# AdeeshKolluru/AdsorbDiff

Measured on AMD Instinct MI355X. Metric: sampled adsorbate sites/sec (50 denoise steps, ~200-atom slabs), higher is better.
Workload: dtype f32 (f16x3-split MFMA, fp32 accumulate; ADF_GEMM=f32 selects exact f32)

## Files before the change

adsorbdiff_amd/csrc/api.hip:

```cpp
#include <stdarg.h>
#include <stdlib.h>
#include <string.h>

#include <new>

#include "common.h"

static thread_local char g_err[512] = "";

void adf_set_error(const char* fmt, ...) {
    va_list ap;
    va_start(ap, fmt);
    vsnprintf(g_err, sizeof(g_err), fmt, ap);
    va_end(ap);
}

extern "C" const char* adf_last_error(void) { return g_err; }
extern "C" const char* adf_version(void) { return "adsorbdiff_hip 0.5.0 (gfx950)"; }

void adf_prof_begin(adf_painn* h, int cat, hipStream_t s) {
    if (!h->prof_on) return;
    if (h->prof_used + 2 > h->prof_ev->size()) {
        for (int i = 0; i < 512; ++i) {
            hipEvent_t e;
            if (hipEventCreate(&e) != hipSuccess) return;
            h->prof_ev->push_back(e);
        }
    }
    h->prof_cat->push_back(cat);
    (void)hipEventRecord((*h->prof_ev)[h->prof_used], s);
    h->prof_used += 1;
}
void adf_prof_end(adf_painn* h, hipStream_t s) {
    if (!h->prof_on || (h->prof_used & 1) == 0) return;
    (void)hipEventRecord((*h->prof_ev)[h->prof_used], s);
    h->prof_used += 1;
}

extern "C" int32_t adf_profile_enable(adf_painn_t h, int32_t on) {
    if (!h) { adf_set_error("null handle"); return ADF_EINVAL; }
    h->prof_on = on != 0;
    h->prof_used = 0;
    h->prof_cat->clear();
    ADF_HIP_CHECK(hipMemset(h->kcount, 0, 8 * sizeof(unsigned long long)));
    return ADF_OK;
}

extern "C" int32_t adf_profile_read(adf_painn_t h, float* ms, int64_t* count, int64_t* message_ksteps, void* stream) {
    if (!h || !ms || !count) { adf_set_error("null argument"); return ADF_EINVAL; }
    ADF_HIP_CHECK(hipStreamSynchronize((hipStream_t)stream));
    if (message_ksteps) {
        unsigned long long k[8];
        ADF_HIP_CHECK(hipMemcpy(k, h->kcount, sizeof(k), hipMemcpyDeviceToHost));
        ADF_HIP_CHECK(hipMemset(h->kcount, 0, sizeof(k)));
        *message_ksteps = (int64_t)k[0];
    }
    for (int c = 0; c < ADF_PROF_NCAT; ++c) { ms[c] = 0.f; count[c] = 0; }
    const size_t pairs = h->prof_used / 2;
    for (size_t i = 0; i < pairs; ++i) {
        float t = 0.f;
        ADF_HIP_CHECK(hipEventElapsedTime(&t, (*h->prof_ev)[2 * i], (*h->prof_ev)[2 * i + 1]));
        const int c = (*h->prof_cat)[i];
        ms[c] += t;
        count[c] += 1;
    }
    h->prof_used = 0;
    h->prof_cat->clear();
    return ADF_OK;
}

template <typename T>
static int32_t dev_alloc(T** p, size_t count) {
    if (*p) { (void)hipFree(*p); *p = nullptr; }
    if (count == 0) return ADF_OK;
    hipError_t e = hipMalloc(reinterpret_cast<void**>(p), count * sizeof(T));
    if (e != hipSuccess) {
        *p = nullptr;
        (void)hipGetLastError();
        adf_set_error("hipMalloc of %zu bytes failed: %s", count * sizeof(T), hipGetErrorString(e));
        return ADF_EOOM;
    }
    return ADF_OK;
}

extern "C" int32_t adf_painn_create(const adf_painn_hparams* hp, adf_painn_t* out) {
    if (!hp || !out) { adf_set_error("null argument"); return ADF_EINVAL; }
    if (hp->hidden_channels % ADF_SLICE_CH != 0 || hp->hidden_channels < 128 || hp->hidden_channels > 1024) {
        adf_set_error("hidden_channels=%d must be a multiple of %d in [128,1024]", hp->hidden_channels, ADF_SLICE_CH);
        return ADF_EINVAL;
    }
    if (hp->num_rbf % 2 != 0 || hp->num_rbf > 128 || hp->num_rbf < 2) {
        adf_set_error("num_rbf=%d must be even and <= 128", hp->num_rbf);
        return ADF_EINVAL;
    }
    if (hp->max_neighbors < 1 || hp->max_neighbors > ADF_MAX_K) {
        adf_set_error("max_neighbors=%d must be in [1,%d]", hp->max_neighbors, ADF_MAX_K);
        return ADF_EINVAL;
    }
    if (hp->num_layers < 1 || hp->num_layers > 16 || hp->num_heads < 0 || hp->num_heads > 2) {
        adf_set_error("num_layers must be in [1,16], num_heads in [0,2]");
        return ADF_EINVAL;
    }
    adf_painn* h = new (std::nothrow) adf_painn();
    if (!h) { adf_set_error("host allocation failed"); return ADF_EOOM; }
    memset(h, 0, sizeof(*h));
    h->hp = *hp;
    h->prof_ev = new std::vector<hipEvent_t>();
    h->prof_cat = new std::vector<int>();
    hipDeviceProp_t prop;
    if (hipGetDevice(&h->device) != hipSuccess || hipGetDeviceProperties(&prop, h->device) != hipSuccess) {
        adf_set_error("no usable HIP device: %s", hipGetErrorString(hipGetLastError()));
        adf_painn_destroy(h);
        return ADF_EHIP;
    }
    h->num_cus = prop.multiProcessorCount;
    h->dist_floor = 1.0e-3f;
    {
        const char* e = getenv("ADF_INCREMENTAL");
        h->inc_on = !(e && e[0] == '0');
        const char* e2 = getenv("ADF_INC_SYNC");
        h->inc_sync = e2 && e2[0] == '1';
    }
    const int H = hp->hidden_channels, R = hp->num_rbf, L = hp->num_layers;
    int32_t st = dev_alloc(&h->rbf_pack, (size_t)L * (H / ADF_SLICE_CH) * R * 192);
    if (st == ADF_OK) st = dev_alloc(&h->rbf_bias_pack, (size_t)L * (H / ADF_SLICE_CH) * 192);
    {
        uint16_t* p16 = nullptr;
        if (st == ADF_OK) st = dev_alloc(&p16, (size_t)L * (H / ADF_SLICE_CH) * R * 192 * 2);
        h->rbf_pack16 = p16;
    }
    if (st == ADF_OK) st = dev_alloc(&h->rbf_bias_pack16, (size_t)L * (H / ADF_SLICE_CH) * 192);
    if (st == ADF_OK) st = dev_alloc(&h->rbf_scales, 16);
    if (st == ADF_OK) st = dev_alloc(&h->flags, ADF_NFLAGS);
    if (st == ADF_OK && hipMemset(h->flags, 0, sizeof(int32_t) * ADF_NFLAGS) != hipSuccess) st = ADF_EHIP;
    {
        const size_t HH = (size_t)H * H;
        const size_t per_layer = HH + 3 * HH + 2 * HH + 2 * HH + 3 * HH;
        const size_t per_head = HH + HH / 2 + 2 * HH + HH + HH / 4 + HH / 2;
        const size_t elems = (size_t)L * per_layer + (size_t)hp->num_heads * per_head;
        h->w16_bytes = elems * 2 * sizeof(uint16_t) + 4096;
        if (st == ADF_OK) st = dev_alloc(&h->w16_arena, h->w16_bytes);
        if (st == ADF_OK) st = dev_alloc(&h->w16_scales, 256);
        if (st == ADF_OK) st = dev_alloc(&h->w16_bias_perm, (size_t)L * 2 * 3 * H);
        if (st == ADF_OK) st = dev_alloc(&h->w16_scratch, 1);
        if (st == ADF_OK) st = dev_alloc(&h->wfrag_arena, h->w16_bytes);
        {
            const char* ef = getenv("ADF_FUSED_MLP");
            h->fused_mlp = ef ? atoi(ef) : 0;
            if (h->fused_mlp < 0 || h->fused_mlp > 2) h->fused_mlp = 0;
        }
        const char* e = getenv("ADF_GEMM");
        h->gemm_f32 = e && strcmp(e, "f32") == 0;
        const char* el = getenv("ADF_LIFT");
        h->lift_on = !(el && strcmp(el, "0") == 0);
        const char* e2 = getenv("ADF_MSG");
        h->msg_f32 = e2 ? strcmp(e2, "f32") == 0 : h->gemm_f32;
    }
    if (st == ADF_OK) st = dev_alloc(&h->kcount, 8);
    if (st == ADF_OK && hipMemset(h->kcount, 0, 8 * sizeof(unsigned long long)) != hipSuccess) st = ADF_EHIP;
    if (st != ADF_OK) { adf_painn_destroy(h); return st; }
    *out = h;
    return ADF_OK;
}

static void inc_free(adf_painn* h) {
    for (int l = 0; l <= ADF_MAX_LAYERS; ++l) {
        if (h->incX[l]) (void)hipFree(h->incX[l]);
        if (h->incV[l]) (void)hipFree(h->incV[l]);
        if (l < ADF_MAX_LAYERS && h->incR[l]) (void)hipFree(h->incR[l]);
        h->incX[l] = h->incV[l] = nullptr;
        if (l < ADF_MAX_LAYERS) h->incR[l] = nullptr;
    }
    void* ptrs[] = {h->inc_c0, h->inc_chg, h->inc_pend, h->inc_need, h->inc_tf, h->inc_list, h->inc_cnt, h->inc_tmp};
    for (void* p : ptrs)
        if (p) (void)hipFree(p);
    h->inc_c0 = h->inc_chg = h->inc_pend = h->inc_need = h->inc_tf = nullptr;
    h->inc_list = h->inc_cnt = nullptr; h->inc_tmp = nullptr; h->inc_tmp_bytes = 0;
    h->inc_capN = 0; h->inc_valid = false;
}

static void free_workspaces(adf_painn* h) {
    void* ptrs[] = {h->nbr_cnt, h->nbr_src, h->nbr_shift, h->deg, h->nptr, h->cursor, h->img_cnt, h->sys_slow, h->scan_tmp,
                    h->e_src, h->e_geom, h->x, h->vecA, h->vecB, h->y, h->xh, h->vv, h->cat, h->dot, h->sys, h->rec, h->lift.buf, h->mag_a, h->mag_b, h->mag_v3,
                    h->cache_d2, h->cache_cid, h->cache_cnt, h->prev_nptr, h->prev_src, h->prev_geom};
    for (void* p : ptrs)
        if (p) (void)hipFree(p);
    h->prev_nptr = h->prev_src = nullptr; h->prev_geom = nullptr; h->inc_valid = false;
    h->nbr_cnt = h->nbr_src = h->nbr_shift = h->deg = h->nptr = h->cursor = h->img_cnt = h->sys_slow = h->e_src = nullptr;
    h->scan_tmp = nullptr; h->scan_tmp_bytes = 0;
    h->e_geom = nullptr;
    h->x = h->vecA = h->vecB = h->y = h->xh = h->vv = h->cat = h->dot = h->sys = h->rec = nullptr;
    h->lift.buf = h->mag_a = h->mag_b = h->mag_v3 = nullptr; h->lift.cap = 0; h->mag_v3_valid = false;
    h->cache_d2 = nullptr; h->cache_cid = nullptr; h->cache_cnt = nullptr; h->cache_valid = false;
    h->capN = h->capB = h->capE = 0;
}

extern "C" int32_t adf_painn_destroy(adf_painn_t h) {
    if (!h) return ADF_OK;
    free_workspaces(h);
    if (h->rbf_pack) (void)hipFree(h->rbf_pack);
    if (h->rbf_bias_pack) (void)hipFree(h->rbf_bias_pack);
    if (h->rec0) (void)hipFree(h->rec0);
    inc_free(h);
    if (h->inc_cnt_host) (void)hipHostFree(h->inc_cnt_host);
    for (int i = 0; i < 2; ++i)
        if (h->inc_ev[i]) (void)hipEventDestroy((hipEvent_t)h->inc_ev[i]);
    if (h->sub_x) (void)hipFree(h->sub_x);
    if (h->sub_vec) (void)hipFree(h->sub_vec);
    if (h->sub_f) (void)hipFree(h->sub_f);
    if (h->rbf_pack16) (void)hipFree(h->rbf_pack16);
    if (h->rbf_bias_pack16) (void)hipFree(h->rbf_bias_pack16);
    if (h->rbf_scales) (void)hipFree(h->rbf_scales);
    if (h->flags) (void)hipFree(h->flags);
    if (h->kcount) (void)hipFree(h->kcount);
    if (h->w16_arena) (void)hipFree(h->w16_arena);
    if (h->wfrag_arena) (void)hipFree(h->wfrag_arena);
    if (h->w16_scales) (void)hipFree(h->w16_scales);
    if (h->w16_bias_perm) (void)hipFree(h->w16_bias_perm);
    if (h->w16_scratch) (void)hipFree(h->w16_scratch);
    if (h->oe0_buf) (void)hipFree(h->oe0_buf);
    if (h->prof_ev) { for (hipEvent_t e : *h->prof_ev) (void)hipEventDestroy(e); delete h->prof_ev; }
    delete h->prof_cat;
    delete h;
    return ADF_OK;
}

extern "C" int32_t adf_painn_set_weights(adf_painn_t h, int32_t n_weights, const void* const* w,
                                         const float* scale_factors, void* stream) {
    if (!h || !w || !scale_factors) { adf_set_error("null argument"); return ADF_EINVAL; }
    const int L = h->hp.num_layers;
    const int expect = 2 + ADF_WEIGHTS_PER_LAYER * L + ADF_WEIGHTS_PER_HEAD * h->hp.num_heads;
    if (n_weights != expect) {
        adf_set_error("expected %d weight tensors, got %d", expect, n_weights);
        return ADF_EINVAL;
    }
    for (int i = 0; i < n_weights; ++i)
        if (!w[i]) { adf_set_error("weight %d is null", i); return ADF_EINVAL; }
    auto f = [&](int i) { return reinterpret_cast<const float*>(w[i]); };
    h->emb = f(0);
    h->rbf_offset = f(1);
    int k = 2;
    for (int l = 0; l < L; ++l) {
        adf_layer_weights& lw = h->layer[l];
        lw.ln_w = f(k++); lw.ln_b = f(k++); lw.xp0_w = f(k++); lw.xp0_b = f(k++); lw.xp2_w = f(k++); lw.xp2_b = f(k++);
        lw.rbf_w = f(k++); lw.rbf_b = f(k++); lw.vp_w = f(k++); lw.xv0_w = f(k++); lw.xv0_b = f(k++);
        lw.xv2_w = f(k++); lw.xv2_b = f(k++);
        h->scale[l] = scale_factors[l];
    }
    for (int hd = 0; hd < h->hp.num_heads; ++hd)
        for (int b = 0; b < 2; ++b) {
            adf_block_weights& bw = h->head[hd][b];
            bw.vec1_w = f(k++); bw.vec2_w = f(k++); bw.un0_w = f(k++); bw.un0_b = f(k++); bw.un2_w = f(k++);
            bw.un2_b = f(k++);
        }
    ADF_TRY(adf_pack_rbf(h, (hipStream_t)stream));
    {
        hipStream_t s = (hipStream_t)stream;
        const long long H = h->hp.hidden_channels, HH = H * H;
        unsigned char* cur = h->w16_arena;
        unsigned char* fcur = h->wfrag_arena;
        int nscale = 0;
        float* bperm = h->w16_bias_perm;
        auto split = [&](const float* w, long long rows, long long K, adf_w16* out, const float* fused_bias = nullptr,
                         bool pair_perm = false) -> int32_t {
            const long long n = rows * K;
            out->hi = cur; cur += n * 2;
            out->lo = cur; cur += n * 2;
            out->inv_scale = h->w16_scales + nscale++;
            out->bias_perm = nullptr;
            out->frag = nullptr;
            if (fused_bias) {
                out->bias_perm = bperm; bperm += 3 * H;
                ADF_TRY(adf_split_weight(w, n, out, h->w16_scratch, s, (int)H, (int)H, fused_bias));
            } else if (pair_perm) {
                ADF_TRY(adf_split_weight(w, n, out, h->w16_scratch, s, (int)H, (int)H, nullptr, 2));
            } else {
                ADF_TRY(adf_split_weight(w, n, out, h->w16_scratch, s));
            }
            if (rows % 32 == 0 && K % 16 == 0) {
                out->frag = fcur; fcur += n * 4;
                ADF_TRY(adf_pack_frag(out, (int)rows, (int)K, out->frag, s));
            }
            return ADF_OK;
        };
        for (int l = 0; l < L; ++l) {
            adf_layer_weights& lw = h->layer[l];
            ADF_TRY(split(lw.xp0_w, H, H, &lw.xp0_16));
            ADF_TRY(split(lw.xp2_w, 3 * H, H, &lw.xp2_16, lw.xp2_b));
            ADF_TRY(split(lw.vp_w, 2 * H, H, &lw.vp_16, nullptr, true));
            ADF_TRY(split(lw.xv0_w, H, 2 * H, &lw.xv0_16));
            ADF_TRY(split(lw.xv2_w, 3 * H, H, &lw.xv2_16, lw.xv2_b));
        }
        for (int hd = 0; hd < h->hp.num_heads; ++hd) {
            adf_block_weights& b0 = h->head[hd][0];
            adf_block_weights& b1 = h->head[hd][1];
            ADF_TRY(split(b0.vec1_w, H, H, &b0.vec1_16));
            ADF_TRY(split(b0.vec2_w, H / 2, H, &b0.vec2_16));
            ADF_TRY(split(b0.un0_w, H, 2 * H, &b0.un0_16));
            ADF_TRY(split(b0.un2_w, H, H, &b0.un2_16));
            ADF_TRY(split(b1.vec1_w, H / 2, H / 2, &b1.vec1_16));
            ADF_TRY(split(b1.un0_w, H / 2, H, &b1.un0_16));
        }
        if ((size_t)(cur - h->w16_arena) > h->w16_bytes || (size_t)(fcur - h->wfrag_arena) > h->w16_bytes || nscale > 256) {
            adf_set_error("internal: fp16 weight arena overflow");
            return ADF_EINVAL;
        }
    }
    h->weights_set = true;
    h->rec0_valid = false;
    h->inc_valid = false;
    return ADF_OK;
}

static int32_t ensure_capacity(adf_painn* h, int64_t N, int64_t B) {
    if (N <= h->capN && B <= h->capB) return ADF_OK;
    const int64_t capN = N > h->capN ? N : h->capN;
    const int64_t capB = B > h->capB ? B : h->capB;
    ADF_HIP_CHECK(hipDeviceSynchronize());
    free_workspaces(h);
    const int64_t H = h->hp.hidden_channels, K = h->hp.max_neighbors;
    const int64_t capE = 2 * capN * K;
    int32_t st = ADF_OK;
#define ALLOC(field, count) if (st == ADF_OK) st = dev_alloc(&h->field, (size_t)(count))
    ALLOC(nbr_cnt, capN);
    ALLOC(nbr_src, capN * K);
    ALLOC(nbr_shift, capN * K);
    ALLOC(cache_d2, capN * K);
    ALLOC(cache_cid, capN * K);
    ALLOC(cache_cnt, capN);
    ALLOC(deg, capN + 1);
    ALLOC(nptr, capN + 1);
    ALLOC(cursor, capN);
    ALLOC(img_cnt, capB);
    ALLOC(sys_slow, capB);
    ALLOC(e_src, capE);
    ALLOC(e_geom, capE);
    if (h->inc_on) {
        ALLOC(prev_nptr, capN + 1);
        ALLOC(prev_src, capE);
        ALLOC(prev_geom, capE);
    }
    if (st == ADF_OK) {
        h->scan_tmp_bytes = adf_scan_temp_bytes(capN + 1);
        unsigned char* tmp = nullptr;
        st = dev_alloc(&tmp, h->scan_tmp_bytes + 16);
        h->scan_tmp = tmp;
    }
    ALLOC(x, capN * H);
    ALLOC(vecA, capN * 3 * H);
    ALLOC(vecB, capN * 3 * H);
    ALLOC(rec, (capN + 1) * 5 * H);
    ALLOC(y, capN * H);
    ALLOC(xh, capN * 3 * H);
    ALLOC(vv, capN * 6 * H);
    ALLOC(cat, capN * 2 * H);
    ALLOC(dot, capN * H);
    ALLOC(sys, capB * 16);
    ALLOC(lift.buf, capN * 3);
    ALLOC(mag_a, capN);
    ALLOC(mag_b, capN);
    ALLOC(mag_v3, capN * 3);
#undef ALLOC
    h->lift.cap = st == ADF_OK ? capN * 3 : 0;
    if (st != ADF_OK) { free_workspaces(h); return st; }
    h->capN = capN; h->capB = capB; h->capE = capE;
    return ADF_OK;
}

static int32_t check_batch(const adf_painn* h, const adf_batch* b) {
    if (!h || !b) { adf_set_error("null argument"); return ADF_EINVAL; }
    if (b->num_atoms <= 0 || b->num_systems <= 0) { adf_set_error("empty batch"); return ADF_EINVAL; }
    if (!b->pos || !b->cell || !b->batch || !b->atom_offset) { adf_set_error("null batch array"); return ADF_EINVAL; }
    for (int k = 0; k < 3; ++k)
        if (b->reps[k] < 0 || b->reps[k] > 16) { adf_set_error("reps[%d]=%d out of range", k, b->reps[k]); return ADF_EINVAL; }
    return ADF_OK;
}

static int32_t read_flags(adf_painn* h, hipStream_t s) {
    int32_t f[ADF_NFLAGS];
    ADF_HIP_CHECK(hipMemcpyAsync(f, h->flags, sizeof(f), hipMemcpyDeviceToHost, s));
    ADF_HIP_CHECK(hipMemsetAsync(h->flags, 0, sizeof(f), s));
    ADF_HIP_CHECK(hipStreamSynchronize(s));
    if (f[4]) { adf_set_error("atomic number outside [1, %d] (rows of the embedding table)", h->hp.num_elements); return ADF_EINVAL; }
    if (f[0]) { adf_set_error("a centre atom has more than %d in-cutoff candidates", ADF_MAX_CAND); return ADF_EOVERFLOW; }
    if (f[2]) { adf_set_error("edge buffer overflow"); return ADF_EOVERFLOW; }
    if (f[3]) { adf_set_error("an atom has more than %d incoming edges", ADF_MAX_INDEG); return ADF_EOVERFLOW; }
    if (f[1]) { adf_set_error("An image has no neighbors"); return ADF_ENONEIGHBOR; }
    if (f[5]) {
        adf_set_error("non-finite model output%s", h->gemm_f32 ? " (exact-f32 arithmetic: the inputs or weights are not finite)"
                      : " in f16x3 arithmetic: an activation left the fp16 range or the inputs are not finite; "
                        "adf_painn_set_arithmetic(h, 1) selects exact f32");
        return ADF_ENUMERIC;
    }
    return ADF_OK;
}

extern "C" int32_t adf_graph_set_moving(adf_painn_t h, const int32_t* moving, const int32_t* mov_idx,
                                        const int32_t* mov_off) {
    if (!h) { adf_set_error("null handle"); return ADF_EINVAL; }
    if (moving && (!mov_idx || !mov_off)) { adf_set_error("moving mask needs mov_idx and mov_off"); return ADF_EINVAL; }
    h->moving = moving; h->mov_idx = mov_idx; h->mov_off = mov_off;
    ADF_HIP_CHECK(hipMemset(h->flags, 0, sizeof(int32_t) * ADF_NFLAGS));
    h->cache_valid = false;
    h->rec0_valid = false;
    h->inc_valid = false;
    return ADF_OK;
}

extern "C" int32_t adf_graph_build(adf_painn_t h, const adf_batch* b, void* stream, int64_t* num_edges) {
    ADF_TRY(check_batch(h, b));
    ADF_TRY(ensure_capacity(h, b->num_atoms, b->num_systems));
    hipStream_t s = (hipStream_t)stream;
    ADF_TRY(adf_graph_build_impl(h, b, s));
    if (num_edges) {
        int32_t e = 0;
        ADF_HIP_CHECK(hipMemcpyAsync(&e, h->nptr + b->num_atoms, sizeof(int32_t), hipMemcpyDeviceToHost, s));
        ADF_TRY(read_flags(h, s));
        *num_edges = e;
    }
    return ADF_OK;
}

__global__ void adf_export_edges_kernel(const int32_t* nptr, const int32_t* e_src, const float4* eg, int N,
                                        int32_t* src, int32_t* dst, float* dist, float* vec, long long cap) {
    const int n = blockIdx.x * 4 + (threadIdx.x >> 6);
    if (n >= N) return;
    for (int e = nptr[n] + (threadIdx.x & 63); e < nptr[n + 1]; e += 64) {
        if (e >= cap) continue;
        if (src) src[e] = e_src[e];
        if (dst) dst[e] = n;
        const float4 q = eg[e];
        if (dist) dist[e] = q.w;
        if (vec) { vec[3 * (size_t)e] = q.x; vec[3 * (size_t)e + 1] = q.y; vec[3 * (size_t)e + 2] = q.z; }
    }
}

__global__ void adf_export_shift_kernel(const int32_t* nbr_shift, int32_t* out, long long n, int r0, int r1, int r2) {
    const long long i = (long long)blockIdx.x * blockDim.x + threadIdx.x;
    if (i >= n) return;
    const int c = nbr_shift[i];
    const int n2 = 2 * r2 + 1, n1 = 2 * r1 + 1;
    const int ia = c / (n1 * n2), rem = c - ia * (n1 * n2);
    out[3 * i] = ia - r0;
    out[3 * i + 1] = rem / n2 - r1;
    out[3 * i + 2] = rem % n2 - r2;
}

extern "C" int32_t adf_graph_export(adf_painn_t h, int32_t* nbr_count, int32_t* nbr_src, int32_t* nbr_shift,
                                    int64_t edge_capacity, int32_t* edge_src, int32_t* edge_dst, float* edge_dist,
                                    float* edge_vec, int64_t* num_edges, void* stream) {
    if (!h || h->lastN <= 0) { adf_set_error("no graph built"); return ADF_EINVAL; }
    hipStream_t s = (hipStream_t)stream;
    const int64_t N = h->lastN, K = h->hp.max_neighbors;
    if (nbr_count) ADF_HIP_CHECK(hipMemcpyAsync(nbr_count, h->nbr_cnt, sizeof(int32_t) * N, hipMemcpyDeviceToDevice, s));
    if (nbr_src) ADF_HIP_CHECK(hipMemcpyAsync(nbr_src, h->nbr_src, sizeof(int32_t) * N * K, hipMemcpyDeviceToDevice, s));
    if (nbr_shift)
        hipLaunchKernelGGL(adf_export_shift_kernel, dim3((unsigned)((N * K + 255) / 256)), dim3(256), 0, s, h->nbr_shift,
                           nbr_shift, (long long)(N * K), h->last_reps[0], h->last_reps[1], h->last_reps[2]);
    if (edge_src || edge_dst || edge_dist || edge_vec)
        hipLaunchKernelGGL(adf_export_edges_kernel, dim3((unsigned)((N + 3) / 4)), dim3(256), 0, s, h->nptr, h->e_src,
                           h->e_geom, (int)N, edge_src, edge_dst, edge_dist, edge_vec, (long long)edge_capacity);
    ADF_HIP_CHECK(hipGetLastError());
    int32_t e = 0;
    ADF_HIP_CHECK(hipMemcpyAsync(&e, h->nptr + N, sizeof(int32_t), hipMemcpyDeviceToHost, s));
    ADF_HIP_CHECK(hipStreamSynchronize(s));
    if (num_edges) *num_edges = e;
    return ADF_OK;
}

static int32_t zero_pad_rows(adf_painn* h, int N, hipStream_t s) {
    const size_t row = (size_t)5 * h->hp.hidden_channels;
    ADF_HIP_CHECK(hipMemsetAsync(h->rec + (size_t)N * row, 0, sizeof(float) * row, s));
    return ADF_OK;
}

static bool use_fused_mlp(const adf_painn* h, int rows) {
    if (h->hp.hidden_channels != 512 || h->gemm_f32 || h->fused_mlp == 0) return false;
    if (h->fused_mlp == 1) return true;
    return rows >= 2 * 64 * h->num_cus;
}

static int32_t make_records(adf_painn* h, int l, int n, const float* x, const float* vec, bool vec_is_zero, float* rec,
                            const int32_t* row_map, hipStream_t s) {
    const int H = h->hp.hidden_channels;
    const adf_layer_weights& w = h->layer[l];
    if (n <= 0) return ADF_OK;
    adf_prof_begin(h, ADF_PROF_NODE, s);
    const bool lift = h->lift_on && !h->gemm_f32;
    static int emit = -1;
    if (emit < 0) { const char* e = getenv("ADF_LIFT_EMIT"); emit = (e && atoi(e) == 0) ? 0 : 1; }
    const bool em = lift && emit;
    ADF_TRY(adf_nodewise_layernorm(x, w.ln_w, w.ln_b, h->y, n, H, s, em ? h->mag_a : nullptr, h->rows_dev));
    if (use_fused_mlp(h, n) && (em || !lift)) {
        adf_epi ep = {};
        ep.vec_in = vec; ep.rec = rec ? rec : h->rec; ep.H = H; ep.vec_is_zero = vec_is_zero ? 1 : 0;
        ep.row_map = row_map; ep.m_dev = h->rows_dev; ep.lift_y = lift ? 1 : 0;
        ep.rec_rows = row_map ? (long long)h->inc_capN : (long long)n;
        ADF_TRY(adf_launch_mlp16(h->y, nullptr, H, em ? h->mag_a : nullptr, w.xp0_16.frag, &w.xp0_16, w.xp0_b, w.xp2_16.frag, &w.xp2_16, n,
                                 H, 1, &ep, s));
        adf_prof_end(h, s);
        return ADF_OK;
    }
    ADF_TRY(adf_linear(h, h->y, H, w.xp0_w, &w.xp0_16, w.xp0_b, h->cat, H, n, H, H, 1, s, em ? h->mag_a : nullptr,
                       em ? h->mag_b : nullptr));
    if (h->gemm_f32) {
        if (row_map) { adf_set_error("internal: mapped records need the f16x3 path"); return ADF_EINVAL; }
        ADF_TRY(adf_launch_gemm(h->cat, H, w.xp2_w, H, w.xp2_b, h->xh, 3 * H, n, 3 * H, H, 0, s));
        ADF_TRY(adf_pack_records(h, n, h->xh, vec, vec_is_zero, s, rec));
    } else {
        adf_epi ep = {};
        ep.vec_in = vec; ep.rec = rec ? rec : h->rec; ep.H = H; ep.vec_is_zero = vec_is_zero ? 1 : 0;
        ep.row_map = row_map;
        ep.rmag = em ? h->mag_b : nullptr;
        ep.m_dev = h->rows_dev;
        ADF_TRY(adf_launch_gemm16_fused(h->cat, H, &w.xp2_16, n, H, H, 1, &ep, s, lift ? &h->lift : nullptr));
    }
    adf_prof_end(h, s);
    return ADF_OK;
}

static int32_t message_layer(adf_painn* h, int l, int N, const float* x, const float* vec, float* x_out,
                             float* vec_out, bool vec_is_zero, hipStream_t s, const int32_t* tlist = nullptr,
                             int n_targets = 0, float* rec = nullptr, bool records_ready = false) {
    if (!records_ready) ADF_TRY(make_records(h, l, N, x, vec, vec_is_zero, rec, nullptr, s));
    adf_prof_begin(h, ADF_PROF_MESSAGE, s);
    const int32_t st = adf_message_impl(h, l, N, x, h->xh, vec, x_out, vec_out, vec_is_zero, s, tlist, n_targets, rec,
                                        tlist ? h->rows_dev : nullptr);
    adf_prof_end(h, s);
    return st;
}

static int32_t update_layer(adf_painn* h, int l, int N, float* x, float* vec, hipStream_t s) {
    const int H = h->hp.hidden_channels;
    const adf_layer_weights& w = h->layer[l];
    adf_prof_begin(h, ADF_PROF_NODE, s);
    if (h->gemm_f32) {
        ADF_TRY(adf_launch_gemm(vec, H, w.vp_w, H, nullptr, h->vv, 2 * H, 3 * N, 2 * H, H, 0, s));
        ADF_TRY(adf_nodewise_update_prep(h->vv, x, h->cat, h->dot, N, H, s));
        ADF_TRY(adf_linear(h, h->cat, 2 * H, w.xv0_w, &w.xv0_16, w.xv0_b, h->y, H, N, H, 2 * H, 1, s));
    } else {
        adf_epi ep = {};
        ep.v1 = h->vv; ep.dotw = h->dot; ep.cat = h->cat; ep.H = H; ep.m_dev = h->rows_dev;
        const adf_lift* lf = h->lift_on ? &h->lift : nullptr;
        ADF_TRY(adf_launch_gemm16_fused(vec, H, &w.vp_16, N, H, H, 3, &ep, s, lf));
        if (use_fused_mlp(h, N)) {
            const float* rm = nullptr;
            if (lf) {
                if (N > lf->cap) { adf_set_error("mlp16: lift scratch holds %lld rows, need %d", lf->cap, N); return ADF_EINVAL; }
                ADF_TRY(adf_launch_rowmag(x, H, H, h->cat, H, N, lf->buf, s, h->rows_dev, 1));
                rm = lf->buf;
            }
            adf_epi e2 = {};
            e2.x = x; e2.vec = vec; e2.dot = h->dot; e2.vv = h->vv; e2.scale = h->scale[l]; e2.H = H;
            e2.m_dev = h->rows_dev; e2.lift_y = h->lift_on ? 1 : 0;
            const int32_t stf = adf_launch_mlp16(x, h->cat, H, rm, w.xv0_16.frag, &w.xv0_16, w.xv0_b, w.xv2_16.frag, &w.xv2_16, N, H, 2, &e2, s);
            adf_prof_end(h, s);
            return stf;
        }
        ADF_TRY(adf_launch_gemm16(x, H, &w.xv0_16, w.xv0_b, h->y, H, N, H, 2 * H, 1, s, h->cat, H, lf, nullptr,
                                  h->lift_on ? h->mag_b : nullptr, h->rows_dev));
    }
    int32_t st;
    if (h->gemm_f32) {
        ADF_TRY(adf_launch_gemm(h->y, H, w.xv2_w, H, w.xv2_b, h->xh, 3 * H, N, 3 * H, H, 0, s));
        st = adf_nodewise_update_apply(h->xh, h->dot, h->vv, x, vec, h->scale[l], N, H, s);
    } else {
        adf_epi ep = {};
        ep.x = x; ep.vec = vec; ep.dot = h->dot; ep.vv = h->vv; ep.scale = h->scale[l]; ep.H = H;
        ep.rmag = h->lift_on ? h->mag_b : nullptr;
        ep.m_dev = h->rows_dev;
        st = adf_launch_gemm16_fused(h->y, H, &w.xv2_16, N, H, H, 2, &ep, s);
    }
    adf_prof_end(h, s);
    return st;
}

extern "C" int32_t adf_painn_message_layer(adf_painn_t h, int32_t layer, int32_t N, const float* x, const float* vec,
                                           float* x_out, float* vec_out, void* stream) {
    if (!h || !h->weights_set || layer < 0 || layer >= h->hp.num_layers || N != h->lastN) {
        adf_set_error("message_layer: bad handle/layer, or N differs from the built graph");
        return ADF_EINVAL;
    }
    hipStream_t s = (hipStream_t)stream;
    ADF_TRY(zero_pad_rows(h, N, s));
    ADF_TRY(message_layer(h, layer, N, x, vec, x_out, vec_out, false, s));
    return ADF_OK;
}

extern "C" int32_t adf_painn_update_layer(adf_painn_t h, int32_t layer, int32_t N, float* x, float* vec, void* stream) {
    if (!h || !h->weights_set || layer < 0 || layer >= h->hp.num_layers) {
        adf_set_error("update_layer: bad handle/layer");
        return ADF_EINVAL;
    }
    ADF_TRY(ensure_capacity(h, N, 1));
    return update_layer(h, layer, N, x, vec, (hipStream_t)stream);
}

__global__ void adf_scatter_rows3_kernel(const float* __restrict__ src, const int32_t* __restrict__ idx, int n,
                                         float* __restrict__ dst) {
    const int i = blockIdx.x * blockDim.x + threadIdx.x;
    if (i < 3 * n) dst[(size_t)idx[i / 3] * 3 + i % 3] = src[i];
}

static int32_t forward_impl(adf_painn_t h, const adf_batch* b, const int32_t* out_idx, int32_t n_out, float* f1,
                            float* f2, void* stream, bool head1_only = false);

extern "C" int32_t adf_painn_forward(adf_painn_t h, const adf_batch* b, float* f1, float* f2, void* stream) {
    return forward_impl(h, b, nullptr, 0, f1, f2, stream);
}

extern "C" int32_t adf_painn_forward_subset(adf_painn_t h, const adf_batch* b, const int32_t* out_idx, int32_t n_out,
                                            float* f1, float* f2, void* stream) {
    if (!out_idx || n_out < 0) { adf_set_error("forward_subset: null index list"); return ADF_EINVAL; }
    return forward_impl(h, b, out_idx, n_out, f1, f2, stream);
}

static int inc_prepare(adf_painn* h, int N) {
    const int L = h->hp.num_layers, H = h->hp.hidden_channels;
    if (!h->inc_on || !h->moving || h->gemm_f32 || h->msg_f32 || L > ADF_MAX_LAYERS || !h->prev_nptr)
        return 0;
    if (N > h->inc_capN) {
        (void)hipDeviceSynchronize();
        inc_free(h);
        const size_t cap = (size_t)N;
        int32_t st = ADF_OK;
        for (int l = 0; l <= L && st == ADF_OK; ++l) {
            st = dev_alloc(&h->incX[l], cap * H);
            if (st == ADF_OK && l >= 1) st = dev_alloc(&h->incV[l], cap * 3 * H);
            if (st == ADF_OK && l < L) st = dev_alloc(&h->incR[l], (cap + 1) * 5 * H);
        }
        if (st == ADF_OK) st = dev_alloc(&h->inc_c0, cap);
        if (st == ADF_OK) st = dev_alloc(&h->inc_chg, 2 * cap);
        if (st == ADF_OK) st = dev_alloc(&h->inc_pend, cap * L);
        if (st == ADF_OK) st = dev_alloc(&h->inc_need, cap * L);
        if (st == ADF_OK) st = dev_alloc(&h->inc_tf, cap * L);
        if (st == ADF_OK) st = dev_alloc(&h->inc_list, cap * L);
        if (st == ADF_OK) st = dev_alloc(&h->inc_cnt, (size_t)2 * ADF_MAX_LAYERS + 1);
        if (st == ADF_OK) {
            h->inc_tmp_bytes = adf_inc_temp_bytes((int64_t)cap);
            unsigned char* tmp = nullptr;
            st = dev_alloc(&tmp, h->inc_tmp_bytes + 16);
            h->inc_tmp = tmp;
        }
        if (st == ADF_OK && !h->inc_cnt_host &&
            hipHostMalloc(reinterpret_cast<void**>(&h->inc_cnt_host), sizeof(int32_t) * 2 * (2 * ADF_MAX_LAYERS + 1)) != hipSuccess)
            st = ADF_EOOM;
        for (int i = 0; i < 2 && st == ADF_OK; ++i)
            if (!h->inc_ev[i] && hipEventCreateWithFlags(reinterpret_cast<hipEvent_t*>(&h->inc_ev[i]), hipEventDisableTiming) != hipSuccess)
                st = ADF_EHIP;
        if (st != ADF_OK) {
            (void)hipGetLastError();
            inc_free(h);
            h->inc_on = false;
            fprintf(stderr, "adsorbdiff_hip: no memory for incremental layers (%d atoms), continuing without\n", N);
            return 0;
        }
        h->inc_capN = (int64_t)cap;
    }
    if (h->inc_N != N || h->inc_layers != L || h->build_serial != h->inc_serial) h->inc_valid = false;
    h->inc_N = N; h->inc_layers = L;
    int32_t* tn = h->nptr; h->nptr = h->prev_nptr; h->prev_nptr = tn;
    int32_t* ts = h->e_src; h->e_src = h->prev_src; h->prev_src = ts;
    float4* tg = h->e_geom; h->e_geom = h->prev_geom; h->prev_geom = tg;
    const int state = h->inc_valid ? 1 : 2;
    h->inc_valid = false;
    return state;
}

__global__ void adf_scatter_rows3_kernel(const float* __restrict__ src, const int32_t* __restrict__ idx, int n,
                                         float* __restrict__ dst);

static int32_t inc_harvest(adf_painn* h, int slot, bool wait, bool peek = false) {
    if (!h->inc_ev_live[slot]) return ADF_OK;
    hipEvent_t ev = (hipEvent_t)h->inc_ev[slot];
    if (wait) {
        ADF_HIP_CHECK(hipEventSynchronize(ev));
    } else {
        const hipError_t q = hipEventQuery(ev);
        if (q == hipErrorNotReady) { (void)hipGetLastError(); return ADF_OK; }
        ADF_HIP_CHECK(q);
    }
    const int L = h->inc_layers, N = h->inc_pend_N[slot];
    const int32_t* c = h->inc_cnt_host + (size_t)slot * (2 * ADF_MAX_LAYERS + 1);
    for (int i = 0; i < 2 * L + 1; ++i) h->inc_seen[i] = c[i];
    h->inc_seen_valid = true;
    h->inc_pend_Nseen = N;
    if (peek) return ADF_OK;
    h->inc_ev_live[slot] = false;
    for (int l = 0; l < L; ++l) {
        const bool whole = h->inc_pend_whole[slot][l] != 0;
        h->inc_rows += (unsigned long long)(whole ? N : c[l]);
        h->inc_rows_full += (unsigned long long)N;
        h->inc_edges += (unsigned long long)(whole ? c[2 * L] : c[L + l]);
        if (whole || c[l] > 0) ++h->inc_launches;
    }
    return ADF_OK;
}

static int32_t forward_incremental(adf_painn* h, int N, const int32_t* Z, const int32_t* out_idx, int32_t n_out,
                                   float* f1, float* f2, bool first, int heads, hipStream_t s) {
    const int L = h->hp.num_layers, H = h->hp.hidden_channels;
    const size_t cap = (size_t)h->inc_capN, row = (size_t)5 * H;
    if (out_idx && n_out == 0) return ADF_OK;
    adf_prof_begin(h, ADF_PROF_GRAPH, s);
    if (first) {
        ADF_TRY(adf_nodewise_embed(h, Z, N, h->incX[0], s));
        for (int l = 0; l < L; ++l) ADF_HIP_CHECK(hipMemsetAsync(h->incR[l] + (size_t)N * row, 0, sizeof(float) * row, s));
        ADF_HIP_CHECK(hipMemsetAsync(h->inc_pend, 0, cap * L, s));
    } else {
        ADF_TRY(adf_inc_compare(h, N, s));
    }
    ADF_HIP_CHECK(hipMemsetAsync(h->inc_cnt, 0, sizeof(int32_t) * (2 * ADF_MAX_LAYERS + 1), s));
    if (out_idx) ADF_TRY(adf_inc_need_from_list(h, N, L, out_idx, n_out, s));
    for (int l = 0; l < L; ++l) ADF_TRY(adf_inc_plan_layer(h, l, N, first, out_idx != nullptr, s));
    ADF_HIP_CHECK(hipMemcpyAsync(h->inc_cnt + 2 * L, h->nptr + N, sizeof(int32_t), hipMemcpyDeviceToDevice, s));
    const int slot = h->inc_slot;
    h->inc_slot ^= 1;
    if (h->inc_ev_live[slot]) ADF_TRY(inc_harvest(h, slot, true));
    int32_t* host = h->inc_cnt_host + (size_t)slot * (2 * ADF_MAX_LAYERS + 1);
    ADF_HIP_CHECK(hipMemcpyAsync(host, h->inc_cnt, sizeof(int32_t) * (2 * L + 1), hipMemcpyDeviceToHost, s));
    ADF_HIP_CHECK(hipEventRecord((hipEvent_t)h->inc_ev[slot], s));
    h->inc_ev_live[slot] = true;
    h->inc_pend_N[slot] = N;
    ADF_TRY(inc_harvest(h, slot ^ 1, false));
    if (h->inc_sync) ADF_TRY(inc_harvest(h, slot, true, true));
    adf_prof_end(h, s);
    if (first) ADF_TRY(make_records(h, 0, N, h->incX[0], nullptr, true, h->incR[0], nullptr, s));
    for (int l = 0; l < L; ++l) {
        const int n_seen = h->inc_seen_valid ? h->inc_seen[l] : N;
        const bool whole = first || !h->inc_seen_valid || h->inc_pend_Nseen != N || (long long)n_seen * 10 >= (long long)N * 9;
        h->inc_pend_whole[slot][l] = whole ? 1 : 0;
        if (h->inc_sync && !whole && n_seen == 0) continue;
        const float* vin = l == 0 ? h->vecA : h->incV[l];
        if (whole) {
            ADF_TRY(message_layer(h, l, N, h->incX[l], vin, h->incX[l + 1], h->incV[l + 1], l == 0, s, nullptr, 0,
                                  h->incR[l], true));
            ADF_TRY(update_layer(h, l, N, h->incX[l + 1], h->incV[l + 1], s));
            if (l + 1 < L)
                ADF_TRY(make_records(h, l + 1, N, h->incX[l + 1], h->incV[l + 1], false, h->incR[l + 1], nullptr, s));
            continue;
        }
        const int32_t* list = h->inc_list + cap * l;
        const int ncap = h->inc_sync ? n_seen : N;
        h->rows_dev = h->inc_cnt + l;
        int32_t st = message_layer(h, l, N, h->incX[l], vin, h->x, h->vecB, l == 0, s, list, ncap, h->incR[l], true);
        if (st == ADF_OK) st = update_layer(h, l, ncap, h->x, h->vecB, s);
        if (st == ADF_OK) {
            adf_prof_begin(h, ADF_PROF_NODE, s);
            st = adf_inc_scatter_rows(h->x, list, ncap, H, h->incX[l + 1], s, h->rows_dev);
            if (st == ADF_OK) st = adf_inc_scatter_rows(h->vecB, list, ncap, 3 * H, h->incV[l + 1], s, h->rows_dev);
            adf_prof_end(h, s);
        }
        if (st == ADF_OK && l + 1 < L) st = make_records(h, l + 1, ncap, h->x, h->vecB, false, h->incR[l + 1], list, s);
        h->rows_dev = nullptr;
        ADF_TRY(st);
    }
    adf_prof_begin(h, ADF_PROF_HEADS, s);
    if (!out_idx) {
        if (heads >= 1) ADF_TRY(adf_head_forward(h, 0, N, h->incX[L], h->incV[L], f1, s));
        if (heads == 2) ADF_TRY(adf_head_forward(h, 1, N, h->incX[L], h->incV[L], f2, s));
        h->x_last = h->incX[L];
    } else {
        if (n_out > h->capS) {
            const int64_t c = (int64_t)n_out + n_out / 4 + 64;
            if (h->sub_x) (void)hipFree(h->sub_x);
            if (h->sub_vec) (void)hipFree(h->sub_vec);
            if (h->sub_f) (void)hipFree(h->sub_f);
            h->sub_x = h->sub_vec = h->sub_f = nullptr; h->capS = 0;
            ADF_TRY(dev_alloc(&h->sub_x, (size_t)c * H));
            ADF_TRY(dev_alloc(&h->sub_vec, (size_t)c * 3 * H));
            ADF_TRY(dev_alloc(&h->sub_f, (size_t)c * 3));
            h->capS = c;
        }
        ADF_TRY(adf_inc_gather_rows(h->incX[L], out_idx, n_out, H, h->sub_x, s));
        ADF_TRY(adf_inc_gather_rows(h->incV[L], out_idx, n_out, 3 * H, h->sub_vec, s));
        for (int hd = 0; hd < heads; ++hd) {
            ADF_TRY(adf_head_forward(h, hd, n_out, h->sub_x, h->sub_vec, h->sub_f, s));
            hipLaunchKernelGGL(adf_scatter_rows3_kernel, dim3((3 * n_out + 255) / 256), dim3(256), 0, s, h->sub_f, out_idx,
                               n_out, hd == 0 ? f1 : f2);
        }
        ADF_HIP_CHECK(hipGetLastError());
    }
    adf_prof_end(h, s);
    h->inc_valid = true;
    return ADF_OK;
}

static int32_t forward_impl(adf_painn_t h, const adf_batch* b, const int32_t* out_idx, int32_t n_out, float* f1,
                            float* f2, void* stream, bool head1_only) {
    ADF_TRY(check_batch(h, b));
    if (!h->weights_set) { adf_set_error("weights not set"); return ADF_EINVAL; }
    const int heads = head1_only ? 1 : h->hp.num_heads;
    if (heads > h->hp.num_heads) { adf_set_error("the model has no force head"); return ADF_EINVAL; }
    if (!b->atomic_numbers || (heads >= 1 && !f1) || (heads == 2 && !f2)) { adf_set_error("null argument"); return ADF_EINVAL; }
    h->x_last = nullptr;
    hipStream_t s = (hipStream_t)stream;
    const int N = b->num_atoms;
    ADF_TRY(ensure_capacity(h, N, b->num_systems));
    const int inc = inc_prepare(h, N);
    adf_prof_begin(h, ADF_PROF_GRAPH, s);
    ADF_TRY(adf_graph_build_impl(h, b, s));
    adf_prof_end(h, s);
    if (inc) {
        h->inc_serial = h->build_serial;
        return forward_incremental(h, N, b->atomic_numbers, out_idx, n_out, f1, f2, inc == 2, heads, s);
    }
    ADF_TRY(zero_pad_rows(h, N, s));
    ADF_TRY(adf_nodewise_embed(h, b->atomic_numbers, N, h->x, s));
    float* vin = h->vecA;
    float* vout = h->vecB;
    const int L = h->hp.num_layers, H = h->hp.hidden_channels;
    float* rec0 = nullptr;
    bool rec0_ready = false;
    if (h->moving) {
        const size_t row = (size_t)5 * H;
        if ((int64_t)N + 1 > h->rec0_cap) {
            if (h->rec0) { (void)hipFree(h->rec0); h->rec0 = nullptr; }
            h->rec0_cap = 0; h->rec0_valid = false;
            ADF_TRY(dev_alloc(&h->rec0, ((size_t)N + 1) * row));
            h->rec0_cap = (int64_t)N + 1;
        }
        rec0 = h->rec0;
        rec0_ready = h->rec0_valid && h->rec0_N == N;
        if (!rec0_ready) ADF_HIP_CHECK(hipMemsetAsync(rec0 + (size_t)N * row, 0, sizeof(float) * row, s));
        h->rec0_valid = true; h->rec0_N = N;
    }
    if (!out_idx) {
        for (int l = 0; l < L; ++l) {
            if (l == 0) ADF_TRY(message_layer(h, 0, N, h->x, vin, h->x, vout, true, s, nullptr, 0, rec0, rec0_ready));
            else
            ADF_TRY(message_layer(h, l, N, h->x, vin, h->x, vout, l == 0, s));
            ADF_TRY(update_layer(h, l, N, h->x, vout, s));
            float* t = vin; vin = vout; vout = t;
        }
        adf_prof_begin(h, ADF_PROF_HEADS, s);
        if (heads >= 1) ADF_TRY(adf_head_forward(h, 0, N, h->x, vin, f1, s));
        if (heads == 2) ADF_TRY(adf_head_forward(h, 1, N, h->x, vin, f2, s));
        adf_prof_end(h, s);
        h->x_last = h->x;
        return ADF_OK;
    }
    if (n_out == 0) return ADF_OK;
    if (n_out > h->capS) {
        const int64_t cap = (int64_t)n_out + n_out / 4 + 64;
        if (h->sub_x) (void)hipFree(h->sub_x);
        if (h->sub_vec) (void)hipFree(h->sub_vec);
        if (h->sub_f) (void)hipFree(h->sub_f);
        h->sub_x = h->sub_vec = h->sub_f = nullptr; h->capS = 0;
        ADF_TRY(dev_alloc(&h->sub_x, (size_t)cap * H));
        ADF_TRY(dev_alloc(&h->sub_vec, (size_t)cap * 3 * H));
        ADF_TRY(dev_alloc(&h->sub_f, (size_t)cap * 3));
        h->capS = cap;
    }
    for (int l = 0; l + 1 < L; ++l) {
        if (l == 0) ADF_TRY(message_layer(h, 0, N, h->x, vin, h->x, vout, true, s, nullptr, 0, rec0, rec0_ready));
        else
        ADF_TRY(message_layer(h, l, N, h->x, vin, h->x, vout, l == 0, s));
        ADF_TRY(update_layer(h, l, N, h->x, vout, s));
        float* t = vin; vin = vout; vout = t;
    }
    ADF_TRY(message_layer(h, L - 1, N, h->x, vin, h->sub_x, h->sub_vec, L == 1, s, out_idx, n_out,
                          L == 1 ? rec0 : nullptr, L == 1 && rec0_ready));
    ADF_TRY(update_layer(h, L - 1, n_out, h->sub_x, h->sub_vec, s));
    adf_prof_begin(h, ADF_PROF_HEADS, s);
    for (int hd = 0; hd < heads; ++hd) {
        ADF_TRY(adf_head_forward(h, hd, n_out, h->sub_x, h->sub_vec, h->sub_f, s));
        hipLaunchKernelGGL(adf_scatter_rows3_kernel, dim3((3 * n_out + 255) / 256), dim3(256), 0, s, h->sub_f, out_idx,
                           n_out, hd == 0 ? f1 : f2);
    }
    ADF_HIP_CHECK(hipGetLastError());
    adf_prof_end(h, s);
    return ADF_OK;
}

extern "C" int32_t adf_painn_set_energy_head(adf_painn_t h, int32_t n_weights, const void* const* w, void* stream) {
    if (!h || !w) { adf_set_error("null argument"); return ADF_EINVAL; }
    if (n_weights != 4) { adf_set_error("set_energy_head: expected 4 tensors (out_energy.0.weight/bias, out_energy.2.weight/bias), got %d", n_weights); return ADF_EINVAL; }
    for (int i = 0; i < 4; ++i)
        if (!w[i]) { adf_set_error("energy-head tensor %d is null", i); return ADF_EINVAL; }
    const int H = h->hp.hidden_channels, H2 = H / 2;
    const size_t n = (size_t)H2 * H;
    if (!h->oe0_buf) ADF_TRY(dev_alloc(&h->oe0_buf, n * 4 + 64));
    h->oe0_w = reinterpret_cast<const float*>(w[0]);
    h->oe0_b = reinterpret_cast<const float*>(w[1]);
    h->oe2_w = reinterpret_cast<const float*>(w[2]);
    h->oe2_b = reinterpret_cast<const float*>(w[3]);
    adf_w16& e = h->oe0_16;
    e = adf_w16{};
    e.hi = h->oe0_buf; e.lo = h->oe0_buf + n * 2; e.inv_scale = reinterpret_cast<float*>(h->oe0_buf + n * 4);
    ADF_TRY(adf_split_weight(h->oe0_w, (long long)n, &e, reinterpret_cast<unsigned int*>(h->oe0_buf + n * 4 + 16),
                             (hipStream_t)stream));
    h->energy_set = true;
    return ADF_OK;
}

extern "C" int32_t adf_painn_set_distance_floor(adf_painn_t h, float floor) {
    if (!h || !(floor > 0.f)) { adf_set_error("set_distance_floor: null handle or non-positive floor"); return ADF_EINVAL; }
    if (floor != h->dist_floor) {
        h->dist_floor = floor;
        h->cache_valid = false;
        h->rec0_valid = false;
        h->inc_valid = false;
    }
    return ADF_OK;
}

__global__ __launch_bounds__(256) void adf_energy_sum_kernel(const float* __restrict__ y, int H2, const float* __restrict__ w,
                                                             const float* __restrict__ bias, const int32_t* __restrict__ atom_offset,
                                                             float* __restrict__ energy) {
    __shared__ float part[4];
    const int b = blockIdx.x, lane = threadIdx.x & 63, wave = threadIdx.x >> 6;
    const int a0 = atom_offset[b], a1 = atom_offset[b + 1];
    const float b0 = bias[0];
    float acc = 0.f;
    for (int a = a0 + wave; a < a1; a += 4) {
        const float* row = y + (size_t)a * H2;
        float d = 0.f;
        for (int c = lane; c < H2; c += 64) d = fmaf(row[c], w[c], d);
        for (int o = 32; o > 0; o >>= 1) d = __fadd_rn(d, __shfl_xor(d, o, 64));
        acc = __fadd_rn(acc, __fadd_rn(d, b0));
    }
    if (lane == 0) part[wave] = acc;
    __syncthreads();
    if (threadIdx.x == 0) energy[b] = __fadd_rn(__fadd_rn(part[0], part[1]), __fadd_rn(part[2], part[3]));
}

extern "C" int32_t adf_painn_forward_energy(adf_painn_t h, const adf_batch* b, float* energy, float* forces, void* stream) {
    ADF_TRY(check_batch(h, b));
    if (!h->energy_set) { adf_set_error("forward_energy: energy head not set (adf_painn_set_energy_head)"); return ADF_EINVAL; }
    if (!energy || (h->hp.num_heads >= 1 && !forces)) { adf_set_error("forward_energy: null output"); return ADF_EINVAL; }
    if (h->hp.num_heads > 1) { adf_set_error("forward_energy: the S2EF model has one force head"); return ADF_EINVAL; }
    hipStream_t s = (hipStream_t)stream;
    ADF_TRY(forward_impl(h, b, nullptr, 0, forces, nullptr, stream));
    if (!h->x_last) { adf_set_error("internal: no node features after the forward"); return ADF_EINVAL; }
    const int N = b->num_atoms, H = h->hp.hidden_channels, H2 = H / 2;
    adf_prof_begin(h, ADF_PROF_HEADS, s);
    ADF_TRY(adf_linear(h, h->x_last, H, h->oe0_w, &h->oe0_16, h->oe0_b, h->y, H2, N, H2, H, 1, s));
    hipLaunchKernelGGL(adf_energy_sum_kernel, dim3(b->num_systems), dim3(256), 0, s, h->y, H2, h->oe2_w, h->oe2_b,
                       b->atom_offset, energy);
    ADF_HIP_CHECK(hipGetLastError());
    adf_prof_end(h, s);
    return ADF_OK;
}

extern "C" int32_t adf_linear_forward(const float* A, const float* W, const float* bias, float* C, int32_t M,
                                      int32_t N, int32_t K, int32_t act_ssilu, int32_t mode, void* stream) {
    hipStream_t s = (hipStream_t)stream;
    if (!A || !W || !C || M <= 0 || N <= 0 || K <= 0) { adf_set_error("bad argument"); return ADF_EINVAL; }
    if (mode == 0) return adf_launch_gemm(A, K, W, K, bias, C, N, M, N, K, act_ssilu, s);
    unsigned char* buf = nullptr;
    const size_t n = (size_t)N * K;
    ADF_TRY(dev_alloc(&buf, n * 4 + 64));
    adf_w16 w16 = {};
    w16.hi = buf; w16.lo = buf + n * 2; w16.inv_scale = reinterpret_cast<float*>(buf + n * 4);
    unsigned int* scratch = reinterpret_cast<unsigned int*>(buf + n * 4 + 16);
    int32_t st = adf_split_weight(W, (long long)n, &w16, scratch, s);
    float* mags = nullptr;
    const char* el = getenv("ADF_LIFT");
    const bool lift = !(el && strcmp(el, "0") == 0);
    if (st == ADF_OK && lift) st = dev_alloc(&mags, (size_t)M);
    adf_lift lf = {mags, M};
    if (st == ADF_OK) st = adf_launch_gemm16(A, K, &w16, bias, C, N, M, N, K, act_ssilu, s, nullptr, 0, lift ? &lf : nullptr);
    (void)hipStreamSynchronize(s);
    (void)hipFree(buf);
    if (mags) (void)hipFree(mags);
    return st;
}

extern "C" int32_t adf_painn_set_arithmetic(adf_painn_t h, int32_t exact_f32) {
    if (!h) { adf_set_error("null handle"); return ADF_EINVAL; }
    h->gemm_f32 = exact_f32 != 0;
    h->msg_f32 = exact_f32 != 0;
    h->rec0_valid = false;
    h->inc_valid = false;
    return ADF_OK;
}

extern "C" int32_t adf_painn_set_fused_mlp(adf_painn_t h, int32_t mode) {
    if (!h || mode < 0 || mode > 2) { adf_set_error("set_fused_mlp: mode must be 0 (never), 1 (always) or 2 (by size)"); return ADF_EINVAL; }
    h->fused_mlp = mode;
    return ADF_OK;
}

extern "C" int32_t adf_painn_set_incremental(adf_painn_t h, int32_t on) {
    if (!h) { adf_set_error("null handle"); return ADF_EINVAL; }
    if ((on != 0) != h->inc_on) {
        ADF_HIP_CHECK(hipDeviceSynchronize());
        h->inc_on = on != 0;
        if (!h->inc_on) inc_free(h);
        if (h->inc_on && h->capN > 0 && !h->prev_nptr) {
            int32_t st = dev_alloc(&h->prev_nptr, (size_t)h->capN + 1);
            if (st == ADF_OK) st = dev_alloc(&h->prev_src, (size_t)h->capE);
            if (st == ADF_OK) st = dev_alloc(&h->prev_geom, (size_t)h->capE);
            if (st != ADF_OK) { h->inc_on = false; return st; }
        }
    }
    h->inc_valid = false;
    (void)inc_harvest(h, h->inc_slot, true);
    (void)inc_harvest(h, h->inc_slot ^ 1, true);
    h->inc_seen_valid = false;
    h->inc_rows = h->inc_rows_full = h->inc_edges = h->inc_launches = 0;
    return ADF_OK;
}

extern "C" int32_t adf_check_flags(adf_painn_t h, void* stream) {
    if (!h) { adf_set_error("null handle"); return ADF_EINVAL; }
    return read_flags(h, (hipStream_t)stream);
}

static int32_t model_check(void* h, const adf_batch* b) { return check_batch((adf_painn*)h, b); }
static int32_t model_grow(void* h, const adf_batch* b, float** sys) {
    adf_painn* p = (adf_painn*)h;
    ADF_TRY(ensure_capacity(p, b->num_atoms, b->num_systems));
    *sys = p->sys;
    return ADF_OK;
}
static int32_t model_forward(void* h, const adf_batch* b, const int32_t* out_idx, int32_t n_out, float* f1, float* f2,
                             hipStream_t s) {
    return forward_impl((adf_painn*)h, b, out_idx, out_idx ? n_out : 0, f1, f2, s, !f2);
}
static void model_prof(void* h, bool begin, hipStream_t s) {
    if (begin) adf_prof_begin((adf_painn*)h, ADF_PROF_STEPPER, s);
    else adf_prof_end((adf_painn*)h, s);
}
static adf_model model(adf_painn_t h) { return {h, model_check, model_grow, model_forward, model_prof}; }

extern "C" int32_t adf_sde_init_placement(adf_painn_t h, const adf_batch* b, float* pos, const int32_t* tags,
                                          const float* noise, void* stream) {
    return adf_model_init_placement(model(h), b, pos, tags, noise, (hipStream_t)stream);
}

extern "C" int32_t adf_sde_step(adf_painn_t h, const adf_batch* b, float* pos, const int32_t* tags,
                                const int32_t* fixed, const float* f1, const float* f2, const adf_step_coef* coef,
                                const float* z_tr, const float* z_rot, int32_t early_stop_count, int32_t* state,
                                float* dcom, float* drot, void* stream) {
    return adf_model_sde_step(model(h), b, pos, tags, fixed, f1, f2, coef, nullptr, 0, z_tr, z_rot, early_stop_count, state,
                              dcom, drot, (hipStream_t)stream);
}

extern "C" int32_t adf_sde_step_scheduled(adf_painn_t h, const adf_batch* b, float* pos, const int32_t* tags,
                                          const int32_t* fixed, const float* f1, const float* f2,
                                          const adf_step_coef* coefs_dev, int32_t num_steps, const float* z_tr,
                                          const float* z_rot, int32_t early_stop_count, int32_t* state, float* dcom,
                                          float* drot, void* stream) {
    return adf_model_sde_step(model(h), b, pos, tags, fixed, f1, f2, nullptr, coefs_dev, num_steps, z_tr, z_rot,
                              early_stop_count, state, dcom, drot, (hipStream_t)stream);
}

extern "C" int32_t adf_sample(adf_painn_t h, const adf_batch* b, float* pos, const int32_t* tags, const int32_t* fixed,
                              const adf_step_coef* coefs_dev, int32_t num_steps, const float* z_tr_all,
                              const float* z_rot_all, int32_t early_stop_count, int32_t poll_every, int32_t* state,
                              const int32_t* out_idx, int32_t n_out, float* f1, float* f2, void* stream) {
    return adf_model_sample(model(h), b, pos, tags, fixed, coefs_dev, num_steps, z_tr_all, z_rot_all, early_stop_count,
                            poll_every, state, out_idx, n_out, f1, f2, nullptr, 0, (hipStream_t)stream);
}

extern "C" int32_t adf_sample_traj(adf_painn_t h, const adf_batch* b, float* pos, const int32_t* tags, const int32_t* fixed,
                                   const adf_step_coef* coefs_dev, int32_t num_steps, const float* z_tr_all,
                                   const float* z_rot_all, int32_t early_stop_count, int32_t poll_every, int32_t* state,
                                   const int32_t* out_idx, int32_t n_out, float* f1, float* f2, adf_frames_t sink,
                                   int32_t frame_every, void* stream) {
    if (!sink) { adf_set_error("sample_traj: null sink"); return ADF_EINVAL; }
    return adf_model_sample(model(h), b, pos, tags, fixed, coefs_dev, num_steps, z_tr_all, z_rot_all, early_stop_count,
                            poll_every, state, out_idx, n_out, f1, f2, sink, frame_every, (hipStream_t)stream);
}

extern "C" int32_t adf_tr_step(adf_painn_t h, const adf_batch* b, float* pos, const int32_t* tags, const float* f1,
                               const adf_tr_coef* coef, const adf_tr_coef* coefs_dev, int32_t num_steps, const float* z,
                               int32_t early_stop_count, int32_t* state, float* dcom, void* stream) {
    return adf_model_tr_step(model(h), b, pos, tags, f1, coef, coefs_dev, num_steps, z, early_stop_count, state, dcom,
                             (hipStream_t)stream);
}

extern "C" int32_t adf_tr_sample(adf_painn_t h, const adf_batch* b, float* pos, const int32_t* tags,
                                 const adf_tr_coef* coefs_dev, int32_t num_steps, const float* z_all,
                                 int32_t early_stop_count, int32_t poll_every, int32_t* state, const int32_t* out_idx,
                                 int32_t n_out, float* f1, void* stream) {
    return adf_model_tr_sample(model(h), b, pos, tags, coefs_dev, num_steps, z_all, early_stop_count, poll_every, state,
                               out_idx, n_out, f1, nullptr, 0, (hipStream_t)stream);
}

extern "C" int32_t adf_tr_sample_traj(adf_painn_t h, const adf_batch* b, float* pos, const int32_t* tags,
                                      const adf_tr_coef* coefs_dev, int32_t num_steps, const float* z_all,
                                      int32_t early_stop_count, int32_t poll_every, int32_t* state, const int32_t* out_idx,
                                      int32_t n_out, float* f1, adf_frames_t sink, int32_t frame_every, void* stream) {
    if (!sink) { adf_set_error("tr_sample_traj: null sink"); return ADF_EINVAL; }
    return adf_model_tr_sample(model(h), b, pos, tags, coefs_dev, num_steps, z_all, early_stop_count, poll_every, state,
                               out_idx, n_out, f1, sink, frame_every, (hipStream_t)stream);
}

extern "C" int32_t adf_get_counters(adf_painn_t h, adf_counters* out, void* stream) {
    if (!h || !out || h->lastN <= 0) { adf_set_error("no forward has run"); return ADF_EINVAL; }
    hipStream_t s = (hipStream_t)stream;
    const int64_t N = h->lastN, H = h->hp.hidden_channels, R = h->hp.num_rbf, L = h->hp.num_layers;
    int32_t e = 0;
    ADF_HIP_CHECK(hipMemcpyAsync(&e, h->nptr + N, sizeof(int32_t), hipMemcpyDeviceToHost, s));
    ADF_HIP_CHECK(hipStreamSynchronize(s));
    const int64_t E = e;
    out->num_edges = E;
    out->num_atoms = N;
    out->message_bytes_per_layer = E * (3 * H * 4 + 12 + 8) + N * (3 * H * 4 + 3 * H * 4) + N * (H * 4 + 3 * H * 4);
    const int64_t head = 2 * (3 * N * H * H + 3 * N * H * H / 2 + N * 2 * H * H + N * H * H + 3 * N * (H / 2) * (H / 2) +
                              N * H * H / 2);
    out->dense_flops = L * (30 * H * H * N + 2 * R * 3 * H * E) + h->hp.num_heads * head;
    ADF_TRY(inc_harvest(h, h->inc_slot, true));
    ADF_TRY(inc_harvest(h, h->inc_slot ^ 1, true));
    out->inc_rows = (int64_t)h->inc_rows; out->inc_rows_full = (int64_t)h->inc_rows_full;
    out->inc_msg_launches = (int64_t)h->inc_launches; out->inc_msg_edges = (int64_t)h->inc_edges;
    return ADF_OK;
}
```

adsorbdiff_amd/csrc/common.h:

```cpp
#pragma once
#include <hip/hip_runtime.h>
#include <stdint.h>
#include <stdio.h>
#include <string>
#include <vector>

#include "../../include/adsorbdiff_hip.h"

#define ADF_GROUP_NODES 32
#define ADF_SLICE_CH 64
#define ADF_MAX_CAND 1024
#define ADF_MAX_K 128
#define ADF_NFLAGS 8
#define ADF_MAX_INDEG 1024
#define ADF_MAX_LAYERS 16

void adf_set_error(const char* fmt, ...);

#define ADF_HIP_CHECK(expr)                                                             \
    do {                                                                                \
        hipError_t _e = (expr);                                                         \
        if (_e != hipSuccess) {                                                         \
            adf_set_error("%s failed: %s (%s:%d)", #expr, hipGetErrorString(_e),        \
                          __FILE__, __LINE__);                                          \
            return (_e == hipErrorOutOfMemory) ? ADF_EOOM : ADF_EHIP;                   \
        }                                                                               \
    } while (0)

#define ADF_TRY(expr)                     \
    do {                                  \
        int32_t _s = (expr);              \
        if (_s != ADF_OK) return _s;      \
    } while (0)

struct adf_w16 {
    void* hi;
    void* lo;
    float* inv_scale;
    float* bias_perm;
    void* frag;
};
struct adf_epi {
    const float* vec_in;
    float* rec;
    float* x;
    float* vec;
    const float* dot;
    const float* vv;
    float* v1;
    float* dotw;
    float* cat;
    float scale;
    int H;
    int vec_is_zero;
    const float* A2;
    int K1;
    const int32_t* row_map;
    const float* rmag;
    unsigned int* out_mag;
    const int32_t* m_dev;
    int accumulate;
    int lift_y;
    const float* gate;
    int gate_ld;
    long long rec_rows;
};
struct adf_lift {
    float* buf;
    long long cap;
};
struct adf_layer_weights {
    const float *ln_w, *ln_b, *xp0_w, *xp0_b, *xp2_w, *xp2_b, *rbf_w, *rbf_b;
    const float *vp_w, *xv0_w, *xv0_b, *xv2_w, *xv2_b;
    adf_w16 xp0_16, xp2_16, vp_16, xv0_16, xv2_16;
};
struct adf_block_weights {
    const float *vec1_w, *vec2_w, *un0_w, *un0_b, *un2_w, *un2_b;
    adf_w16 vec1_16, vec2_16, un0_16, un2_16;
};

struct adf_painn {
    adf_painn_hparams hp;
    int device;
    bool weights_set;
    const float* emb;
    const float* rbf_offset;
    adf_layer_weights layer[16];
    adf_block_weights head[2][2];
    float scale[16];
    float* rbf_pack;
    float* rbf_bias_pack;
    void* rbf_pack16;
    float* rbf_bias_pack16;
    float* rbf_scales;
    unsigned char* w16_arena;
    size_t w16_bytes;
    float* w16_scales;
    float* w16_bias_perm;
    unsigned int* w16_scratch;
    unsigned char* wfrag_arena;
    int fused_mlp;
    bool gemm_f32;
    bool msg_f32;
    bool lift_on;
    adf_lift lift;
    float *mag_a, *mag_b;
    float* mag_v3;
    bool mag_v3_valid;

    int64_t capN, capB, capE;
    int32_t* nbr_cnt;
    int32_t* nbr_src;
    int32_t* nbr_shift;
    int32_t* deg;
    int32_t* nptr;
    int32_t* cursor;
    int32_t* img_cnt;
    int32_t* sys_slow;
    void* scan_tmp;
    size_t scan_tmp_bytes;
    const int32_t* moving;
    const int32_t* mov_idx;
    const int32_t* mov_off;
    float* cache_d2;
    int32_t* cache_cid;
    int32_t* cache_cnt;
    bool cache_valid;
    int32_t* e_src;
    float4* e_geom;
    int32_t* flags;
    float *x, *vecA, *vecB, *y, *xh, *vv, *cat, *dot;
    float* rec;
    bool rbf_uniform;
    float* rec0;
    int64_t rec0_cap, rec0_N;
    bool rec0_valid;
    bool inc_on;
    bool inc_valid;
    int64_t inc_capN, inc_N;
    int inc_layers;
    float* incX[ADF_MAX_LAYERS + 1];
    float* incV[ADF_MAX_LAYERS + 1];
    float* incR[ADF_MAX_LAYERS];
    int32_t *prev_nptr, *prev_src;
    float4* prev_geom;
    unsigned char *inc_c0, *inc_chg;
    unsigned char *inc_pend, *inc_need, *inc_tf;
    int32_t* inc_list;
    int32_t* inc_cnt;
    int32_t* inc_cnt_host;
    void* inc_ev[2];
    bool inc_ev_live[2];
    int inc_slot;
    bool inc_sync;
    int32_t inc_seen[2 * ADF_MAX_LAYERS + 1];
    bool inc_seen_valid;
    unsigned char inc_pend_whole[2][ADF_MAX_LAYERS];
    int32_t inc_pend_N[2];
    int32_t inc_pend_Nseen;
    const int32_t* rows_dev;
    void* inc_tmp; size_t inc_tmp_bytes;
    unsigned long long inc_rows, inc_rows_full, inc_edges, inc_launches;
    unsigned long long build_serial, inc_serial;
    float *sub_x, *sub_vec, *sub_f;
    int64_t capS;
    float* sys;
    const float *oe0_w, *oe0_b, *oe2_w, *oe2_b;
    adf_w16 oe0_16;
    unsigned char* oe0_buf;
    bool energy_set;
    const float* x_last;
    float dist_floor;
    int64_t lastN, lastB;
    int32_t last_reps[3];
    int num_cus;
    bool prof_on;
    std::vector<hipEvent_t>* prof_ev;
    std::vector<int>* prof_cat;
    size_t prof_used;
    unsigned long long* kcount;
};

enum { ADF_PROF_GRAPH = 0, ADF_PROF_MESSAGE = 1, ADF_PROF_NODE = 2, ADF_PROF_HEADS = 3, ADF_PROF_STEPPER = 4 };
void adf_prof_begin(adf_painn* h, int cat, hipStream_t s);
void adf_prof_end(adf_painn* h, hipStream_t s);

int32_t adf_launch_gemm(const float* A, int lda, const float* W, int ldw, const float* bias, float* C, int ldc,
                        int M, int N, int K, int act_ssilu, hipStream_t s);
int32_t adf_launch_gemm16(const float* A, int lda, const adf_w16* W, const float* bias, float* C, int ldc, int M,
                          int N, int K, int act_ssilu, hipStream_t s, const float* A2 = nullptr, int K1 = 0,
                          const adf_lift* lf = nullptr, const float* premag = nullptr, float* out_mag = nullptr,
                          const int32_t* m_dev = nullptr, int accumulate = 0,
                          const float* gate = nullptr, int gate_ld = 0);
int32_t adf_launch_rowmag(const float* A, int lda, int K1, const float* A2, int K2, long long M, float* mag, hipStream_t s,
                          const int32_t* m_dev = nullptr, int m_mul = 1);
int32_t adf_split_weight(const float* w, long long n, adf_w16* out, unsigned int* scratch_bits, hipStream_t s,
                         int perm_H = 0, int K = 0, const float* bias = nullptr, int parts = 3);
int32_t adf_launch_gemm16_vecnorm(const float* A, int lda, const adf_w16* W, float* nrm, int M, int N, int K,
                                  hipStream_t s, const adf_lift* lf = nullptr, const float* premag = nullptr);
int32_t adf_launch_gemm16_fused(const float* A, int lda, const adf_w16* W, int M, int H, int K, int epi,
                                const adf_epi* ep, hipStream_t s, const adf_lift* lf = nullptr);
static inline int32_t adf_linear(const adf_painn* h, const float* A, int lda, const float* W, const adf_w16* W16,
                                 const float* bias, float* C, int ldc, int M, int N, int K, int act, hipStream_t s,
                                 const float* premag = nullptr, float* out_mag = nullptr) {
    if (h->gemm_f32) return adf_launch_gemm(A, lda, W, K, bias, C, ldc, M, N, K, act, s);
    return adf_launch_gemm16(A, lda, W16, bias, C, ldc, M, N, K, act, s, nullptr, 0, h->lift_on ? &h->lift : nullptr,
                             h->lift_on ? premag : nullptr, h->lift_on ? out_mag : nullptr, h->rows_dev);
}
int32_t adf_pack_frag(const adf_w16* w, int N, int K, void* out, hipStream_t s);
int32_t adf_launch_mlp16(const float* A1, const float* A2, int lda, const float* rmag, const void* W0f, const adf_w16* W0,
                         const float* bias0, const void* W2f, const adf_w16* W2, int M, int H, int epi, const adf_epi* ep,
                         hipStream_t s);
int32_t adf_graph_build_impl(adf_painn* h, const adf_batch* b, hipStream_t s);
size_t adf_inc_temp_bytes(int64_t n);
int32_t adf_inc_compare(adf_painn* h, int N, hipStream_t s);
int32_t adf_inc_need_from_list(adf_painn* h, int N, int L, const int32_t* out_idx, int n_out, hipStream_t s);
int32_t adf_inc_plan_layer(adf_painn* h, int l, int N, bool first, bool have_need, hipStream_t s);
int32_t adf_inc_scatter_rows(const float* src, const int32_t* idx, int n, int width, float* dst, hipStream_t s,
                             const int32_t* n_dev = nullptr);
int32_t adf_inc_gather_rows(const float* src, const int32_t* idx, int n, int width, float* dst, hipStream_t s);
size_t adf_scan_temp_bytes(int64_t n);
int32_t adf_message_impl(adf_painn* h, int layer, int N, const float* x, const float* xh, const float* vec,
                         float* x_out, float* vec_out, bool vec_is_zero, hipStream_t s,
                         const int32_t* tlist = nullptr, int n_targets = 0, const float* rec = nullptr,
                         const int32_t* n_targets_dev = nullptr);
int32_t adf_pack_rbf(adf_painn* h, hipStream_t s);
int32_t adf_pack_rbf_layer(adf_painn* h, int l, hipStream_t s);
int32_t adf_pack_records(adf_painn* h, int N, const float* xh, const float* vec, bool vec_is_zero, hipStream_t s,
                         float* rec = nullptr);
int32_t adf_nodewise_embed(adf_painn* h, const int32_t* Z, int N, float* x, hipStream_t s);
int32_t adf_nodewise_layernorm(const float* x, const float* w, const float* b, float* y, int N, int H, hipStream_t s,
                               float* out_mag = nullptr, const int32_t* n_dev = nullptr);
int32_t adf_nodewise_update_prep(const float* vv, const float* x, float* cat, float* dot, int N, int H, hipStream_t s);
int32_t adf_nodewise_update_apply(const float* h3, const float* dot, const float* vv, float* x, float* vec,
                                  float scale, int N, int H, hipStream_t s);
int32_t adf_head_forward(adf_painn* h, int head, int N, const float* x, const float* vec, float* out, hipStream_t s);
int32_t adf_stepper_init(const adf_batch* b, float* pos, const int32_t* tags, const float* noise,
                         hipStream_t s);
int32_t adf_stepper_step(float* sys, const adf_batch* b, float* pos, const int32_t* tags, const int32_t* fixed,
                         const float* f1, const float* f2, const adf_step_coef* coef, const adf_step_coef* coefs_dev,
                         int num_steps, const float* z_tr, const float* z_rot, int32_t early_stop_count,
                         int32_t* state, float* dcom, float* drot, hipStream_t s);
int32_t adf_stepper_tr_step(float* sys, const adf_batch* b, float* pos, const int32_t* tags, const float* f1,
                            const adf_tr_coef* coef, const adf_tr_coef* coefs_dev, int num_steps, const float* z,
                            int32_t early_stop_count, int32_t* state, float* dcom, hipStream_t s);

struct adf_model {
    void* h;
    int32_t (*check)(void* h, const adf_batch* b);
    int32_t (*grow)(void* h, const adf_batch* b, float** sys);
    int32_t (*forward)(void* h, const adf_batch* b, const int32_t* out_idx, int32_t n_out, float* f1, float* f2,
                       hipStream_t s);
    void (*prof)(void* h, bool begin, hipStream_t s);
};
int32_t adf_frames_push_impl(adf_frames* f, const float* src, hipStream_t s);
int32_t adf_model_init_placement(const adf_model& m, const adf_batch* b, float* pos, const int32_t* tags,
                                 const float* noise, hipStream_t s);
int32_t adf_model_sde_step(const adf_model& m, const adf_batch* b, float* pos, const int32_t* tags, const int32_t* fixed,
                           const float* f1, const float* f2, const adf_step_coef* coef, const adf_step_coef* coefs_dev,
                           int32_t num_steps, const float* z_tr, const float* z_rot, int32_t early_stop_count,
                           int32_t* state, float* dcom, float* drot, hipStream_t s);
int32_t adf_model_tr_step(const adf_model& m, const adf_batch* b, float* pos, const int32_t* tags, const float* f1,
                          const adf_tr_coef* coef, const adf_tr_coef* coefs_dev, int32_t num_steps, const float* z,
                          int32_t early_stop_count, int32_t* state, float* dcom, hipStream_t s);
int32_t adf_model_sample(const adf_model& m, const adf_batch* b, float* pos, const int32_t* tags, const int32_t* fixed,
                         const adf_step_coef* coefs_dev, int32_t num_steps, const float* z_tr_all, const float* z_rot_all,
                         int32_t early_stop_count, int32_t poll_every, int32_t* state, const int32_t* out_idx,
                         int32_t n_out, float* f1, float* f2, adf_frames* sink, int32_t frame_every, hipStream_t s);
int32_t adf_model_tr_sample(const adf_model& m, const adf_batch* b, float* pos, const int32_t* tags,
                            const adf_tr_coef* coefs_dev, int32_t num_steps, const float* z_all, int32_t early_stop_count,
                            int32_t poll_every, int32_t* state, const int32_t* out_idx, int32_t n_out, float* f1,
                            adf_frames* sink, int32_t frame_every, hipStream_t s);
```

adsorbdiff_amd/csrc/gemm16.hip:

```cpp
#include <stdlib.h>

#include "common.h"

typedef float f32x16 __attribute__((ext_vector_type(16)));
typedef _Float16 half8 __attribute__((ext_vector_type(8)));
typedef _Float16 half4 __attribute__((ext_vector_type(4)));

#ifndef EPI_ABL
#define EPI_ABL 0
#endif
#ifndef G16_ABL
#define G16_ABL 0
#endif
#ifndef G16_WDEEP
#define G16_WDEEP 1
#endif
#define HK 32
#define TLD3 96
#define TLD2 64
#define HLD 40

__device__ __forceinline__ float adf_pow2_lift(float mx) {
    if (!(mx > 0.f) || !(mx < 3.0e38f)) return 1.0f;
    int e;
    (void)frexpf(mx, &e);
    e = 15 - e;
    e = e > 120 ? 120 : (e < -120 ? -120 : e);
    return ldexpf(1.0f, e);
}

__device__ __forceinline__ float ssilu16(float x) {
    float s = x / (1.0f + expf(-x));
    return s * 1.6666666666666667f;
}

__device__ __forceinline__ float adf_row16_max(float v) {
#define ADF_ROR(n_) __int_as_float(__builtin_amdgcn_update_dpp(0, __float_as_int(v), 0x120 + (n_), 0xf, 0xf, false))
    v = fmaxf(v, ADF_ROR(8));
    v = fmaxf(v, ADF_ROR(4));
    v = fmaxf(v, ADF_ROR(2));
    v = fmaxf(v, ADF_ROR(1));
#undef ADF_ROR
    return v;
}

template <int ACT, int MI, int NJ, int EPI, bool WR = false, int NWN = 2>
__global__ __launch_bounds__(128 * NWN, (MI == 4 || NWN == 4 ? 1 : 2)) void adf_gemm_f16x3_kernel(
    const float* __restrict__ A, int lda, const _Float16* __restrict__ Whi, const _Float16* __restrict__ Wlo,
    const float* __restrict__ inv_scale, const float* __restrict__ bias, float* __restrict__ C, int ldc, int Mh, int N,
    int K, int tiles_n, adf_epi ep) {
    const int M = ep.m_dev ? min(Mh, (int)*ep.m_dev) : Mh;
    static_assert(NWN == 2 || WR, "eight waves only with the register-streamed weights");
    constexpr int NT = 128 * NWN;
    constexpr int TM = 64 * MI;
    constexpr int TN = 32 * NJ * NWN;
    constexpr int NA = TM * 8 / NT;
    static_assert(TM * 8 % NT == 0, "A staging: whole float4s per thread");
    constexpr int LDS_WR = 4 * TM * HLD > NT / 64 * 6400 ? 4 * TM * HLD : NT / 64 * 6400;
    __shared__ __attribute__((aligned(16))) _Float16 lds[WR ? LDS_WR : (2 * TM + 2 * TN) * HLD];
    __shared__ float rinv[TM];
    _Float16* Ahi = lds;
    _Float16* Alo = Ahi + TM * HLD;
    _Float16* Bhi = Alo + TM * HLD;
    _Float16* Blo = Bhi + TN * HLD;
    const int tid = threadIdx.x;
    const int lane = tid & 63;
    const int wave = tid >> 6;
    const int wm = (wave / NWN) * (32 * MI);
    const int wn = (wave % NWN) * (32 * NJ);

    const int id = blockIdx.x;
    const int xcd = id & 7;
    const int qd = id >> 3;
    const int tile_m = (qd / tiles_n) * 8 + xcd;
    const int tile_n = qd % tiles_n;
    const int m0 = tile_m * (EPI >= 3 ? TM / 3 : TM);
    const int n0 = tile_n * TN;
    if (m0 >= M) return;

    unsigned int a_goff[NA];
    int a_off[NA];
    float a_rs[NA];
    auto global_row = [&](int row) -> unsigned int {
        if constexpr (EPI >= 3) {
            const int atom = m0 + (row / 96) * 32 + (row & 31), ax = (row % 96) >> 5;
            return (unsigned int)min(atom, M - 1) * 3u + ax;
        } else {
            return (unsigned int)min(m0 + row, M - 1);
        }
    };
#pragma unroll
    for (int i = 0; i < NA; ++i) {
        const int f = tid + NT * i;
        const int row = f >> 3, kq = f & 7;
        const unsigned int grow = global_row(row);
        a_goff[i] = (grow * (unsigned int)lda + kq * 4) * 4u;
        a_off[i] = row * HLD + kq * 4;
        a_rs[i] = ep.rmag ? adf_pow2_lift(ep.rmag[grow]) : 1.0f;
    }
    if (tid < TM) rinv[tid] = ep.rmag ? 1.0f / adf_pow2_lift(ep.rmag[global_row(tid)]) : 1.0f;
    const char* const A1b = reinterpret_cast<const char*>(A);
    const char* const A2b = reinterpret_cast<const char*>(ep.A2) - (size_t)ep.K1 * 4;
    int w_src[NJ];
    int w_off[NJ];
#pragma unroll
    for (int i = 0; i < NJ; ++i) {
        const int f = tid + 256 * i;
        const int row = f >> 2, part = f & 3;
        w_src[i] = min(n0 + row, N - 1) * K + part * 8;
        w_off[i] = row * HLD + part * 8;
    }

    float4 ra[NA];
    half8 rwh[NJ], rwl[NJ];
#pragma unroll
    for (int i = 0; i < NA; ++i) ra[i] = *reinterpret_cast<const float4*>(A1b + a_goff[i]);
    if constexpr (!WR) {
#pragma unroll
        for (int i = 0; i < NJ; ++i) {
            rwh[i] = *reinterpret_cast<const half8*>(Whi + w_src[i]);
            rwl[i] = *reinterpret_cast<const half8*>(Wlo + w_src[i]);
        }
    }
    half8 wfa[NJ][2], wfb[NJ][2];
    const half8* const wfr = reinterpret_cast<const half8*>(Whi) + (size_t)((n0 + wn) / 32) * (K / 16) * 128 + lane;
    auto load_wf = [&](int s_, half8 (&wf)[NJ][2]) {
#pragma unroll
        for (int j = 0; j < NJ; ++j) {
            const size_t base = ((size_t)j * (K / 16) + s_) * 128;
            wf[j][0] = wfr[base];
            wf[j][1] = wfr[base + 64];
        }
    };
    if constexpr (WR) load_wf(0, wfa);

    f32x16 acc[MI][NJ];
#pragma unroll
    for (int i = 0; i < MI; ++i)
#pragma unroll
        for (int j = 0; j < NJ; ++j)
#pragma unroll
            for (int r = 0; r < 16; ++r) acc[i][j][r] = 0.f;

    const int nk = K / HK;
    const int fa = (wm + (lane & 31)) * HLD + (lane >> 5) * 8;
    const int fb = (wn + (lane & 31)) * HLD + (lane >> 5) * 8;
    auto stage_a = [&](int boff = 0) {
#pragma unroll
        for (int i = 0; i < NA; ++i) {
            if (G16_ABL & 2) {
                *reinterpret_cast<float2*>(Ahi + boff + a_off[i]) = make_float2(ra[i].x, ra[i].y);
                *reinterpret_cast<float2*>(Alo + boff + a_off[i]) = make_float2(ra[i].z, ra[i].w);
                continue;
            }
            const float sx = ra[i].x * a_rs[i], sy = ra[i].y * a_rs[i], sz = ra[i].z * a_rs[i], sw = ra[i].w * a_rs[i];
            half4 h, l;
            h[0] = (_Float16)sx; h[1] = (_Float16)sy; h[2] = (_Float16)sz; h[3] = (_Float16)sw;
            l[0] = (_Float16)(sx - (float)h[0]); l[1] = (_Float16)(sy - (float)h[1]);
            l[2] = (_Float16)(sz - (float)h[2]); l[3] = (_Float16)(sw - (float)h[3]);
            *reinterpret_cast<half4*>(Ahi + boff + a_off[i]) = h;
            *reinterpret_cast<half4*>(Alo + boff + a_off[i]) = l;
        }
    };
    auto request_a = [&](int kt1) {
        const int k1 = kt1 * HK;
        const char* ab = ((ep.K1 > 0 && k1 >= ep.K1) ? A2b : A1b) + (size_t)k1 * 4;
#pragma unroll
        for (int i = 0; i < NA; ++i) ra[i] = *reinterpret_cast<const float4*>(ab + ((G16_ABL & 4) ? (a_goff[i] & 127u) : a_goff[i]));
    };
    if constexpr (WR) {
        auto kstep = [&](int boff, int ks, const half8 (&cur)[NJ][2]) {
            if (G16_ABL & 8) { asm volatile("" :: "v"(cur[0][0]), "v"(cur[0][1]), "v"(cur[NJ - 1][0]), "v"(cur[NJ - 1][1])); return; }
#pragma unroll
            for (int i = 0; i < MI; ++i) {
                const half8 ah = *reinterpret_cast<const half8*>(Ahi + boff + fa + i * 32 * HLD + ks * 16);
                const half8 al = *reinterpret_cast<const half8*>(Alo + boff + fa + i * 32 * HLD + ks * 16);
#pragma unroll
                for (int j = 0; j < NJ; ++j) {
                    acc[i][j] = __builtin_amdgcn_mfma_f32_32x32x16_f16(al, cur[j][0], acc[i][j], 0, 0, 0);
                    acc[i][j] = __builtin_amdgcn_mfma_f32_32x32x16_f16(ah, cur[j][1], acc[i][j], 0, 0, 0);
                    acc[i][j] = __builtin_amdgcn_mfma_f32_32x32x16_f16(ah, cur[j][0], acc[i][j], 0, 0, 0);
                }
            }
        };
        {
            constexpr int BUF = 2 * TM * HLD;
            float4 rb[NA];
            auto request_b = [&](int kt1) {
                const int k1 = kt1 * HK;
                const char* ab = ((ep.K1 > 0 && k1 >= ep.K1) ? A2b : A1b) + (size_t)k1 * 4;
#pragma unroll
                for (int i = 0; i < NA; ++i) rb[i] = *reinterpret_cast<const float4*>(ab + ((G16_ABL & 4) ? (a_goff[i] & 127u) : a_goff[i]));
            };
            auto stage_from = [&](const float4 (&src)[NA], int boff) {
#pragma unroll
                for (int i = 0; i < NA; ++i) {
                    if (G16_ABL & 2) {
                        *reinterpret_cast<float2*>(Ahi + boff + a_off[i]) = make_float2(src[i].x, src[i].y);
                        *reinterpret_cast<float2*>(Alo + boff + a_off[i]) = make_float2(src[i].z, src[i].w);
                        continue;
                    }
                    const float sx = src[i].x * a_rs[i], sy = src[i].y * a_rs[i], sz = src[i].z * a_rs[i], sw = src[i].w * a_rs[i];
                    half4 h, l;
                    h[0] = (_Float16)sx; h[1] = (_Float16)sy; h[2] = (_Float16)sz; h[3] = (_Float16)sw;
                    l[0] = (_Float16)(sx - (float)h[0]); l[1] = (_Float16)(sy - (float)h[1]);
                    l[2] = (_Float16)(sz - (float)h[2]); l[3] = (_Float16)(sw - (float)h[3]);
                    *reinterpret_cast<half4*>(Ahi + boff + a_off[i]) = h;
                    *reinterpret_cast<half4*>(Alo + boff + a_off[i]) = l;
                }
            };
#if G16_WDEEP
            half8 wfc[NJ][2], wfd[NJ][2];
            load_wf(1, wfb);
            auto tile = [&](int kt, int cur, const float4 (&nxt_regs)[NA], const half8 (&w0)[NJ][2], const half8 (&w1)[NJ][2],
                            half8 (&w2)[NJ][2], half8 (&w3)[NJ][2]) {
                load_wf(min(2 * kt + 2, 2 * nk - 1), w2);
                __builtin_amdgcn_sched_barrier(0);
                kstep(cur, 0, w0);
                __builtin_amdgcn_sched_barrier(0);
                load_wf(min(2 * kt + 3, 2 * nk - 1), w3);
                __builtin_amdgcn_sched_barrier(0);
                kstep(cur, 1, w1);
                stage_from(nxt_regs, BUF - cur);
#else
            auto tile = [&](int kt, int cur, const float4 (&nxt_regs)[NA]) {
                load_wf(2 * kt + 1, wfb);
                __builtin_amdgcn_sched_barrier(0);
                kstep(cur, 0, wfa);
                __builtin_amdgcn_sched_barrier(0);
                load_wf(min(2 * kt + 2, 2 * nk - 1), wfa);
                __builtin_amdgcn_sched_barrier(0);
                kstep(cur, 1, wfb);
                stage_from(nxt_regs, BUF - cur);
#endif
                __builtin_amdgcn_sched_group_barrier(0x100, 2 * MI, 0);
#pragma unroll
                for (int u = 0; u < 3 * MI * NJ; ++u) {
                    __builtin_amdgcn_sched_group_barrier(0x8, 1, 0);
                    __builtin_amdgcn_sched_group_barrier(0x2, 4, 0);
                    if (u % 3 == 2) __builtin_amdgcn_sched_group_barrier(0x200, 1, 0);
                }
                __builtin_amdgcn_sched_barrier(0);
            };
            __syncthreads();
            stage_a(0);
            request_a(min(1, nk - 1));
            request_b(min(2, nk - 1));
            __syncthreads();
            for (int kt = 0; kt < nk; kt += 2) {
#if G16_WDEEP
                tile(kt, 0, ra, wfa, wfb, wfc, wfd);
                request_a(min(kt + 3, nk - 1));
                __syncthreads();
                tile(kt + 1, BUF, rb, wfc, wfd, wfa, wfb);
#else
                tile(kt, 0, ra);
                request_a(min(kt + 3, nk - 1));
                __syncthreads();
                tile(kt + 1, BUF, rb);
#endif
                request_b(min(kt + 4, nk - 1));
                __syncthreads();
            }
        }
    } else {
    for (int kt = 0; kt < nk; ++kt) {
        __syncthreads();
        stage_a();
#pragma unroll
        for (int i = 0; i < NJ; ++i) {
            *reinterpret_cast<half8*>(Bhi + w_off[i]) = rwh[i];
            *reinterpret_cast<half8*>(Blo + w_off[i]) = rwl[i];
        }
        __syncthreads();
        if (kt + 1 < nk) {
            const int k1 = (kt + 1) * HK;
            request_a(kt + 1);
#pragma unroll
            for (int i = 0; i < NJ; ++i) {
                rwh[i] = *reinterpret_cast<const half8*>(Whi + w_src[i] + k1);
                rwl[i] = *reinterpret_cast<const half8*>(Wlo + w_src[i] + k1);
            }
        }
#pragma unroll
        for (int ks = 0; ks < 2; ++ks) {
            half8 bh[NJ], bl[NJ];
#pragma unroll
            for (int j = 0; j < NJ; ++j) {
                bh[j] = *reinterpret_cast<const half8*>(Bhi + fb + j * 32 * HLD + ks * 16);
                bl[j] = *reinterpret_cast<const half8*>(Blo + fb + j * 32 * HLD + ks * 16);
            }
#pragma unroll
            for (int i = 0; i < MI; ++i) {
                const half8 ah = *reinterpret_cast<const half8*>(Ahi + fa + i * 32 * HLD + ks * 16);
                const half8 al = *reinterpret_cast<const half8*>(Alo + fa + i * 32 * HLD + ks * 16);
#pragma unroll
                for (int j = 0; j < NJ; ++j) {
                    acc[i][j] = __builtin_amdgcn_mfma_f32_32x32x16_f16(al, bh[j], acc[i][j], 0, 0, 0);
                    acc[i][j] = __builtin_amdgcn_mfma_f32_32x32x16_f16(ah, bl[j], acc[i][j], 0, 0, 0);
                    acc[i][j] = __builtin_amdgcn_mfma_f32_32x32x16_f16(ah, bh[j], acc[i][j], 0, 0, 0);
                }
            }
        }
    }
    }

    const float isc = *inv_scale;
    if constexpr (EPI == 0) {
        if (((N | ldc) & 3) == 0 && (reinterpret_cast<uintptr_t>(C) & 15) == 0 && NJ % 2 == 0) {
            const int q = lane & 31;
            __syncthreads();
            float* T = reinterpret_cast<float*>(lds) + wave * (32 * TLD2);
#pragma unroll
            for (int jj = 0; jj < NJ / 2; ++jj) {
                const int cb = n0 + wn + 64 * jj;
                const float bv0 = (bias && cb + q < N) ? bias[cb + q] : 0.f;
                const float bv1 = (bias && cb + 32 + q < N) ? bias[cb + 32 + q] : 0.f;
#pragma unroll
                for (int i = 0; i < MI; ++i) {
#pragma unroll
                    for (int r = 0; r < 16; ++r) {
                        const int lr = (r & 3) + 8 * (r >> 2) + 4 * (lane >> 5);
                        const float sc = isc * rinv[wm + 32 * i + lr];
                        float v0 = acc[i][2 * jj][r] * sc + bv0, v1 = acc[i][2 * jj + 1][r] * sc + bv1;
                        if (ACT) { v0 = ssilu16(v0); v1 = ssilu16(v1); }
                        T[lr * TLD2 + q] = v0;
                        T[lr * TLD2 + 32 + q] = v1;
                    }
                    __builtin_amdgcn_fence(__ATOMIC_RELEASE, "wavefront");
                    __builtin_amdgcn_wave_barrier();
#pragma unroll
                    for (int it = 0; it < 8; ++it) {
                        const int item = lane + 64 * it;
                        const int lr = item >> 4, c4 = item & 15;
                        const int row = m0 + wm + 32 * i + lr, col = cb + 4 * c4;
                        float4 v = *reinterpret_cast<const float4*>(T + lr * TLD2 + 4 * c4);
                        if (row < M && col < N) {
                            if (ep.gate) {
                                const float4 g4 = *reinterpret_cast<const float4*>(ep.gate + (size_t)(row / 3) * ep.gate_ld + col);
                                v.x = g4.x * v.x; v.y = g4.y * v.y; v.z = g4.z * v.z; v.w = g4.w * v.w;
                            }
                            if (ep.accumulate) {
                                const float4 o = *reinterpret_cast<const float4*>(C + (size_t)row * ldc + col);
                                v.x += o.x; v.y += o.y; v.z += o.z; v.w += o.w;
                            }
                            *reinterpret_cast<float4*>(C + (size_t)row * ldc + col) = v;
                        }
                        if (ep.out_mag) {
                            float mg = col < N ? fmaxf(fmaxf(fabsf(v.x), fabsf(v.y)), fmaxf(fabsf(v.z), fabsf(v.w))) : 0.f;
                            mg = adf_row16_max(mg);
                            if (c4 == 0 && row < M) atomicMax(ep.out_mag + row, __float_as_uint(mg));
                        }
                    }
                    __builtin_amdgcn_wave_barrier();
                }
            }
            return;
        }
#pragma unroll
        for (int j = 0; j < NJ; ++j) {
            const int col = n0 + wn + 32 * j + (lane & 31);
            if (col >= N) continue;
            const float bv = bias ? bias[col] : 0.f;
#pragma unroll
            for (int i = 0; i < MI; ++i) {
#pragma unroll
                for (int r = 0; r < 16; ++r) {
                    const int row = m0 + wm + 32 * i + (r & 3) + 8 * (r >> 2) + 4 * (lane >> 5);
                    if (row < M) {
                        float v = acc[i][j][r] * (isc * rinv[row - m0]) + bv;
                        if (ACT) v = ssilu16(v);
                        if (ep.accumulate) v += C[(size_t)row * ldc + col];
                        C[(size_t)row * ldc + col] = v;
                        if (ep.out_mag) atomicMax(ep.out_mag + row, __float_as_uint(fabsf(v)));
                    }
                }
            }
        }
    } else if constexpr (EPI == 3) {
        static_assert(EPI != 3 || (NJ == 2 && MI == 3), "vec_proj epilogue: 3 components x (v1, v2)");
        const int q = lane & 31;
        const int g = (n0 + wn) / 64;
        const int H = ep.H;
        const float inv_sqrt_h = 1.0f / sqrtf((float)H);
        __syncthreads();
        float* T = reinterpret_cast<float*>(lds) + wave * 3200;
        const int a0 = m0 + (wave / NWN) * 32;
        float dv[16], nv[16];
#pragma unroll
        for (int r = 0; r < 16; ++r) {
            const int lr = (r & 3) + 8 * (r >> 2) + 4 * (lane >> 5);
            float d = 0.f, qq = 0.f;
#pragma unroll
            for (int i = 0; i < 3; ++i) {
                const float sc = isc * rinv[wm + 32 * i + lr];
                const float v1 = acc[i][0][r] * sc, v2 = acc[i][1][r] * sc;
                d += v1 * v2;
                qq += v2 * v2;
                T[lr * TLD3 + i * 32 + q] = v1;
            }
            dv[r] = d * inv_sqrt_h;
            nv[r] = sqrtf(qq + 1e-8f);
        }
        __builtin_amdgcn_fence(__ATOMIC_RELEASE, "wavefront");
        __builtin_amdgcn_wave_barrier();
#pragma unroll
        for (int it = 0; it < 4; ++it) {
            const int item = lane + 64 * it;
            const int lr = item >> 3, c4 = item & 7;
            const int n = a0 + lr;
            if (n < M) {
                float* vo = ep.v1 + (size_t)n * 3 * H + 32 * g + 4 * c4;
#pragma unroll
                for (int ax = 0; ax < 3; ++ax) {
                    const float4 tv_ = *reinterpret_cast<const float4*>(T + lr * TLD3 + ax * 32 + 4 * c4);
                    if (G16_ABL & 1) asm volatile("" :: "v"(tv_.x), "v"(tv_.w)); else
                    *reinterpret_cast<float4*>(vo + ax * H) = tv_;
                }
            }
        }
        __builtin_amdgcn_wave_barrier();
#pragma unroll
        for (int r = 0; r < 16; ++r) {
            const int lr = (r & 3) + 8 * (r >> 2) + 4 * (lane >> 5);
            T[lr * TLD3 + q] = dv[r];
            T[lr * TLD3 + 32 + q] = nv[r];
        }
        __builtin_amdgcn_fence(__ATOMIC_RELEASE, "wavefront");
        __builtin_amdgcn_wave_barrier();
#pragma unroll
        for (int it = 0; it < 4; ++it) {
            const int lr = it * 8 + (lane >> 3), c4 = lane & 7;
            const int n = a0 + lr, c = 32 * g + 4 * c4;
            if (n < M) {
                const float4 dv_ = *reinterpret_cast<const float4*>(T + lr * TLD3 + 4 * c4);
                const float4 nv_ = *reinterpret_cast<const float4*>(T + lr * TLD3 + 32 + 4 * c4);
                if (G16_ABL & 1) { asm volatile("" :: "v"(dv_.x), "v"(nv_.w)); } else {
                *reinterpret_cast<float4*>(ep.dotw + (size_t)n * H + c) = dv_;
                *reinterpret_cast<float4*>(ep.cat + (size_t)n * H + c) = nv_;
                }
            }
        }
    } else if constexpr (EPI == 4) {
        static_assert(EPI != 4 || (NJ == 2 && MI == 3), "norm epilogue: 3 components x 64 columns per wave");
        const int q = lane & 31;
        const int cb = n0 + wn;
        __syncthreads();
        float* T = reinterpret_cast<float*>(lds) + wave * 3200;
        const int a0 = m0 + (wave / NWN) * 32;
#pragma unroll
        for (int r = 0; r < 16; ++r) {
            const int lr = (r & 3) + 8 * (r >> 2) + 4 * (lane >> 5);
#pragma unroll
            for (int j = 0; j < 2; ++j) {
                const float a = acc[0][j][r] * (isc * rinv[wm + lr]), b = acc[1][j][r] * (isc * rinv[wm + 32 + lr]),
                            d = acc[2][j][r] * (isc * rinv[wm + 64 + lr]);
                T[lr * TLD2 + j * 32 + q] = sqrtf(a * a + b * b + d * d);
            }
        }
        __builtin_amdgcn_fence(__ATOMIC_RELEASE, "wavefront");
        __builtin_amdgcn_wave_barrier();
#pragma unroll
        for (int it = 0; it < 8; ++it) {
            const int lr = it * 4 + (lane >> 4), c4 = lane & 15;
            const int n = a0 + lr, c = cb + 4 * c4;
            if (n < M && c < N)
                *reinterpret_cast<float4*>(ep.cat + (size_t)n * N + c) = *reinterpret_cast<const float4*>(T + lr * TLD2 + 4 * c4);
        }
    } else {
        static_assert(EPI >= 3 || (NJ == 3 && MI == 2), "fused epilogues are written for the 64 x 96 wave tile");
        if (((EPI_ABL & 1) && EPI == 1) || ((EPI_ABL & 2) && EPI == 2)) {
            float sacc = 0.f;
            for (int i = 0; i < MI; ++i) for (int j = 0; j < NJ; ++j) for (int r = 0; r < 16; ++r) sacc += acc[i][j][r];
            if (ep.H < 0) ep.x[0] = sacc;
            return;
        }
        const int q = lane & 31;
        const int g = (n0 + wn) / 96;
        const int H = ep.H;
        const float b0 = bias[n0 + wn + q], b1 = bias[n0 + wn + 32 + q], b2 = bias[n0 + wn + 64 + q];
        __syncthreads();
        float* T = reinterpret_cast<float*>(lds) + wave * 3200;
#pragma unroll
        for (int i = 0; i < MI; ++i) {
#pragma unroll
            for (int r = 0; r < 16; ++r) {
                const int lr = (r & 3) + 8 * (r >> 2) + 4 * (lane >> 5);
                const float sc = isc * rinv[wm + 32 * i + lr];
                T[lr * TLD3 + q] = acc[i][0][r] * sc + b0;
                T[lr * TLD3 + 32 + q] = acc[i][1][r] * sc + b1;
                T[lr * TLD3 + 64 + q] = acc[i][2][r] * sc + b2;
            }
            __builtin_amdgcn_fence(__ATOMIC_RELEASE, "wavefront");
            __builtin_amdgcn_wave_barrier();
            const int c4 = lane & 7;
            const int c = 32 * g + 4 * c4;
            if constexpr (EPI == 1) {
                float4 v0[4], v1[4], v2[4];
                if (EPI_ABL & 4) { for (int it = 0; it < 4; ++it) { v0[it] = make_float4(1.f, 2.f, 3.f, 4.f); v1[it] = v0[it]; v2[it] = v0[it]; } }
                else if (!ep.vec_is_zero) {
#pragma unroll
                    for (int it = 0; it < 4; ++it) {
                        const int n = min(m0 + wm + 32 * i + it * 8 + (lane >> 3), M - 1);
                        const float* vr = ep.vec_in + (size_t)n * 3 * H + c;
                        v0[it] = *reinterpret_cast<const float4*>(vr);
                        v1[it] = *reinterpret_cast<const float4*>(vr + H);
                        v2[it] = *reinterpret_cast<const float4*>(vr + 2 * H);
                    }
                }
#pragma unroll
                for (int it = 0; it < 4; ++it) {
                    const int lr = it * 8 + (lane >> 3);
                    const int n = m0 + wm + 32 * i + lr;
                    const float4 p0 = *reinterpret_cast<const float4*>(T + lr * TLD3 + 4 * c4);
                    const float4 p1 = *reinterpret_cast<const float4*>(T + lr * TLD3 + 32 + 4 * c4);
                    const float4 p2 = *reinterpret_cast<const float4*>(T + lr * TLD3 + 64 + 4 * c4);
                    if ((EPI_ABL & 8) && n >= 0) { if (ep.H < 0) ep.rec[0] = p0.x + p1.x + p2.x + v0[it].x + v1[it].y + v2[it].z; }
                    else if (n < M) {
                        float* rec = ep.rec + ((size_t)(ep.row_map ? ep.row_map[n] : n) * (H / 32) + g) * 160;
                        float4* ra_ = reinterpret_cast<float4*>(rec + 16 * c4);
                        if (!ep.vec_is_zero) {
                            ra_[0] = make_float4(v0[it].x * p1.x, v1[it].x * p1.x, v2[it].x * p1.x, p0.x);
                            ra_[1] = make_float4(v0[it].y * p1.y, v1[it].y * p1.y, v2[it].y * p1.y, p0.y);
                            ra_[2] = make_float4(v0[it].z * p1.z, v1[it].z * p1.z, v2[it].z * p1.z, p0.z);
                            ra_[3] = make_float4(v0[it].w * p1.w, v1[it].w * p1.w, v2[it].w * p1.w, p0.w);
                        } else {
                            ra_[0] = make_float4(0.f, 0.f, 0.f, p0.x);
                            ra_[1] = make_float4(0.f, 0.f, 0.f, p0.y);
                            ra_[2] = make_float4(0.f, 0.f, 0.f, p0.z);
                            ra_[3] = make_float4(0.f, 0.f, 0.f, p0.w);
                        }
                        *reinterpret_cast<float4*>(rec + 128 + 4 * c4) = p2;
                    }
                }
            } else {
                float4 d[4], xv[4], w1[4][3], tv[4][3];
#pragma unroll
                for (int it = 0; it < 4; ++it) {
                    const int n = min(m0 + wm + 32 * i + it * 8 + (lane >> 3), M - 1);
                    const size_t xo = (size_t)n * H + c;
                    d[it] = *reinterpret_cast<const float4*>(ep.dot + xo);
                    xv[it] = *reinterpret_cast<const float4*>(ep.x + xo);
                    const float* vr = ep.vec + (size_t)n * 3 * H + c;
                    const float* v1p = ep.vv + (size_t)n * 3 * H + c;
#pragma unroll
                    for (int ax = 0; ax < 3; ++ax) {
                        w1[it][ax] = *reinterpret_cast<const float4*>(v1p + ax * H);
                        tv[it][ax] = *reinterpret_cast<const float4*>(vr + ax * H);
                    }
                }
#pragma unroll
                for (int it = 0; it < 4; ++it) {
                    const int lr = it * 8 + (lane >> 3);
                    const int n = m0 + wm + 32 * i + lr;
                    const float4 p0 = *reinterpret_cast<const float4*>(T + lr * TLD3 + 4 * c4);
                    const float4 p1 = *reinterpret_cast<const float4*>(T + lr * TLD3 + 32 + 4 * c4);
                    const float4 p2 = *reinterpret_cast<const float4*>(T + lr * TLD3 + 64 + 4 * c4);
                    const float k2 = 0.70710678118654752f, sc = ep.scale;
                    float4 xo4 = xv[it];
                    xo4.x = (xo4.x + (p0.x + p1.x * d[it].x) * k2) * sc;
                    xo4.y = (xo4.y + (p0.y + p1.y * d[it].y) * k2) * sc;
                    xo4.z = (xo4.z + (p0.z + p1.z * d[it].z) * k2) * sc;
                    xo4.w = (xo4.w + (p0.w + p1.w * d[it].w) * k2) * sc;
                    if (n < M) {
                        *reinterpret_cast<float4*>(ep.x + (size_t)n * H + c) = xo4;
                        float* vr = ep.vec + (size_t)n * 3 * H + c;
#pragma unroll
                        for (int ax = 0; ax < 3; ++ax) {
                            float4 t = tv[it][ax];
                            const float4 v1 = w1[it][ax];
                            t.x += p2.x * v1.x; t.y += p2.y * v1.y; t.z += p2.z * v1.z; t.w += p2.w * v1.w;
                            *reinterpret_cast<float4*>(vr + ax * H) = t;
                        }
                    }
                }
            }
            __builtin_amdgcn_wave_barrier();
        }
    }
}

__global__ __launch_bounds__(256) void adf_rowmag_kernel(const float* __restrict__ A, int lda, int K1,
                                                         const float* __restrict__ A2, int K2, long long M,
                                                         float* __restrict__ mag, const int32_t* __restrict__ m_dev,
                                                         int m_mul) {
    const long long r = (long long)blockIdx.x * 4 + (threadIdx.x >> 6);
    const int lane = threadIdx.x & 63;
    if (r >= M || (m_dev && r >= (long long)*m_dev * m_mul)) return;
    float mx = 0.f;
    const float* a = A + (size_t)r * lda;
    for (int k = lane * 4; k < K1; k += 256) {
        const float4 v = *reinterpret_cast<const float4*>(a + k);
        mx = fmaxf(fmaxf(fmaxf(mx, fabsf(v.x)), fabsf(v.y)), fmaxf(fabsf(v.z), fabsf(v.w)));
    }
    if (A2) {
        const float* b = A2 + (size_t)r * lda;
        for (int k = lane * 4; k < K2; k += 256) {
            const float4 v = *reinterpret_cast<const float4*>(b + k);
            mx = fmaxf(fmaxf(fmaxf(mx, fabsf(v.x)), fabsf(v.y)), fmaxf(fabsf(v.z), fabsf(v.w)));
        }
    }
#pragma unroll
    for (int o = 32; o > 0; o >>= 1) mx = fmaxf(mx, __shfl_xor(mx, o));
    if (lane == 0) mag[r] = mx;
}

int32_t adf_launch_rowmag(const float* A, int lda, int K1, const float* A2, int K2, long long M, float* mag, hipStream_t s,
                          const int32_t* m_dev, int m_mul) {
    if (M <= 0) return ADF_OK;
    hipLaunchKernelGGL(adf_rowmag_kernel, dim3((unsigned)((M + 3) / 4)), dim3(256), 0, s, A, lda, K1, A2, K2, M, mag, m_dev,
                       m_mul);
    ADF_HIP_CHECK(hipGetLastError());
    return ADF_OK;
}

static int32_t lift_mags(const float* A, int lda, int K1, const float* A2, int K2, long long rows, const adf_lift* lf,
                         const float* premag, const float** out, hipStream_t s, const int32_t* m_dev = nullptr, int m_mul = 1) {
    *out = premag;
    if (!premag && lf && lf->buf) {
        if (rows > lf->cap) { adf_set_error("gemm16: lift scratch holds %lld rows, need %lld", lf->cap, rows); return ADF_EINVAL; }
        ADF_TRY(adf_launch_rowmag(A, lda, K1, A2, K2, rows, lf->buf, s, m_dev, m_mul));
        *out = lf->buf;
    }
    return ADF_OK;
}

__global__ void adf_absmax_kernel(const float* __restrict__ w, long long n, unsigned int* out_bits) {
    float m = 0.f;
    for (long long i = (long long)blockIdx.x * blockDim.x + threadIdx.x; i < n; i += (long long)gridDim.x * blockDim.x)
        m = fmaxf(m, fabsf(w[i]));
#pragma unroll
    for (int o = 32; o > 0; o >>= 1) m = fmaxf(m, __shfl_xor(m, o));
    if ((threadIdx.x & 63) == 0) atomicMax(out_bits, __float_as_uint(m));
}

__global__ void adf_split_kernel(const float* __restrict__ w, long long n, const unsigned int* absmax_bits,
                                 _Float16* __restrict__ hi, _Float16* __restrict__ lo, float* inv_scale, int perm_H,
                                 int K, const float* __restrict__ bias, float* __restrict__ bias_perm, int parts) {
    const float amax = __uint_as_float(*absmax_bits);
    int e = 0;
    if (amax > 0.f) (void)frexpf(amax, &e);
    const float scale = ldexpf(1.0f, 10 - e);
    if (blockIdx.x == 0 && threadIdx.x == 0) *inv_scale = 1.0f / scale;
    for (long long i = (long long)blockIdx.x * blockDim.x + threadIdx.x; i < n; i += (long long)gridDim.x * blockDim.x) {
        long long src = i;
        if (perm_H > 0) {
            const long long prow = i / K;
            const int k = (int)(i - prow * K);
            const int gw = 32 * parts;
            const int g = (int)(prow / gw), part = (int)((prow % gw) / 32), qq = (int)(prow % 32);
            const long long orow = (long long)part * perm_H + 32 * g + qq;
            src = orow * K + k;
            if (k == 0 && bias_perm) bias_perm[prow] = bias ? bias[orow] : 0.f;
        }
        const float v = w[src] * scale;
        const _Float16 h = (_Float16)v;
        hi[i] = h;
        lo[i] = (_Float16)(v - (float)h);
    }
}

int32_t adf_split_weight(const float* w, long long n, adf_w16* out, unsigned int* scratch_bits, hipStream_t s,
                         int perm_H, int K, const float* bias, int parts) {
    ADF_HIP_CHECK(hipMemsetAsync(scratch_bits, 0, sizeof(unsigned int), s));
    hipLaunchKernelGGL(adf_absmax_kernel, dim3(64), dim3(256), 0, s, w, n, scratch_bits);
    hipLaunchKernelGGL(adf_split_kernel, dim3(64), dim3(256), 0, s, w, n, scratch_bits, (_Float16*)out->hi,
                       (_Float16*)out->lo, out->inv_scale, perm_H, K, bias, out->bias_perm, parts);
    ADF_HIP_CHECK(hipGetLastError());
    return ADF_OK;
}

static int32_t check_a_span(long long rows, int lda) {
    if (rows * (long long)lda * 4 >= (1ll << 32)) {
        adf_set_error("gemm16: A operand of %lld rows x %d exceeds the 32-bit offset range, split the batch", rows, lda);
        return ADF_EOOM;
    }
    return ADF_OK;
}

int32_t adf_launch_gemm16(const float* A, int lda, const adf_w16* W, const float* bias, float* C, int ldc, int M,
                          int N, int K, int act_ssilu, hipStream_t s, const float* A2, int K1, const adf_lift* lf,
                          const float* premag, float* out_mag, const int32_t* m_dev, int accumulate, const float* gate,
                          int gate_ld) {
    if (M <= 0) return ADF_OK;
    if (K % HK != 0 || (lda & 3) || (A2 && (K1 <= 0 || K1 % HK != 0 || K1 >= K))) {
        adf_set_error("gemm16: K=%d (K1=%d) must be multiples of %d and lda a multiple of 4", K, K1, HK);
        return ADF_EINVAL;
    }
    ADF_TRY(check_a_span(M, lda));
    static int mi = 0;
    if (!mi) { const char* e = getenv("ADF_GEMM16_MI"); mi = e ? atoi(e) : 2; if (mi != 4) mi = 2; }
    const int TM = 64 * mi, TN = 256;
    const int tiles_n = (N + TN - 1) / TN;
    const int tiles_m = (M + TM - 1) / TM;
    const int tiles_m8 = (tiles_m + 7) / 8 * 8;
    dim3 grid((unsigned)(tiles_m8 * tiles_n));
    adf_epi ep = {};
    ep.A2 = A2; ep.K1 = A2 ? K1 : 0; ep.m_dev = m_dev; ep.accumulate = accumulate;
    ep.gate = gate; ep.gate_ld = gate_ld;
    if (gate && ((N | ldc) & 3)) { adf_set_error("gemm16: the gate epilogue needs N and ldc multiples of 4"); return ADF_EINVAL; }
    ADF_TRY(lift_mags(A, lda, A2 ? K1 : K, A2, A2 ? K - K1 : 0, M, lf, premag, &ep.rmag, s, m_dev, 1));
    if (out_mag) {
        ADF_HIP_CHECK(hipMemsetAsync(out_mag, 0, sizeof(float) * (size_t)M, s));
        ep.out_mag = reinterpret_cast<unsigned int*>(out_mag);
    }
    static int w8 = -1;
    if (w8 < 0) { const char* e = getenv("ADF_GEMM_W8_PLAIN"); w8 = (e && atoi(e) == 0) ? 0 : 1; }
    static int ncu = 0;
    if (!ncu) { int dev = 0; if (hipGetDevice(&dev) != hipSuccess || hipDeviceGetAttribute(&ncu, hipDeviceAttributeMultiprocessorCount, dev) != hipSuccess || ncu <= 0) ncu = 256; }
    const long long wg8 = (long long)((M + 191) / 192) * (N / 256 > 0 ? N / 256 : 1);
    const bool ragged = wg8 < 4ll * ncu && wg8 % ncu != 0 && wg8 % ncu < (3 * ncu) / 10 && wg8 > ncu;
    if (w8 == 1 && W->frag && N % 256 == 0 && (K / HK) % 2 == 0 && mi == 2 && !ragged) {
        const int tn8 = N / 256, tmw8 = ((M + 191) / 192 + 7) / 8 * 8;
        dim3 g8((unsigned)(tmw8 * tn8));
        if (act_ssilu)
            hipLaunchKernelGGL((adf_gemm_f16x3_kernel<1, 3, 2, 0, true, 4>), g8, dim3(512), 0, s, A, lda, (const _Float16*)W->frag,
                               (const _Float16*)nullptr, W->inv_scale, bias, C, ldc, M, N, K, tn8, ep);
        else
            hipLaunchKernelGGL((adf_gemm_f16x3_kernel<0, 3, 2, 0, true, 4>), g8, dim3(512), 0, s, A, lda, (const _Float16*)W->frag,
                               (const _Float16*)nullptr, W->inv_scale, bias, C, ldc, M, N, K, tn8, ep);
        ADF_HIP_CHECK(hipGetLastError());
        return ADF_OK;
    }
#define LAUNCH16(ACT_, MI_)                                                                                  \
    hipLaunchKernelGGL((adf_gemm_f16x3_kernel<ACT_, MI_, 4, 0>), grid, dim3(256), 0, s, A, lda,              \
                       (const _Float16*)W->hi, (const _Float16*)W->lo, W->inv_scale, bias, C, ldc, M, N, K, \
                       tiles_n, ep)
    if (mi == 4) { if (act_ssilu) LAUNCH16(1, 4); else LAUNCH16(0, 4); }
    else { if (act_ssilu) LAUNCH16(1, 2); else LAUNCH16(0, 2); }
#undef LAUNCH16
    ADF_HIP_CHECK(hipGetLastError());
    return ADF_OK;
}

int32_t adf_launch_gemm16_vecnorm(const float* A, int lda, const adf_w16* W, float* nrm, int M, int N, int K,
                                  hipStream_t s, const adf_lift* lf, const float* premag) {
    if (M <= 0) return ADF_OK;
    if (K % HK != 0 || (lda & 3) || (N & 3)) { adf_set_error("gemm16_vecnorm: bad shape"); return ADF_EINVAL; }
    ADF_TRY(check_a_span(3ll * M, lda));
    adf_epi ep = {};
    ep.cat = nrm;
    ADF_TRY(lift_mags(A, lda, K, nullptr, 0, 3ll * M, lf, premag, &ep.rmag, s));
    const int tn = (N + 127) / 128, tm8 = ((M + 63) / 64 + 7) / 8 * 8;
    static int w8 = -1;
    if (w8 < 0) { const char* e = getenv("ADF_GEMM_W8"); w8 = (e && atoi(e) == 0) ? 0 : 1; }
    if (w8 && W->frag && N % 256 == 0 && (K / HK) % 2 == 0) {
        hipLaunchKernelGGL((adf_gemm_f16x3_kernel<0, 3, 2, 4, true, 4>), dim3((unsigned)(tm8 * (N / 256))), dim3(512), 0, s, A, lda,
                           (const _Float16*)W->frag, (const _Float16*)nullptr, W->inv_scale, (const float*)nullptr,
                           (float*)nullptr, 0, M, N, K, N / 256, ep);
        ADF_HIP_CHECK(hipGetLastError());
        return ADF_OK;
    }
    hipLaunchKernelGGL((adf_gemm_f16x3_kernel<0, 3, 2, 4>), dim3((unsigned)(tm8 * tn)), dim3(256), 0, s, A, lda,
                       (const _Float16*)W->hi, (const _Float16*)W->lo, W->inv_scale, (const float*)nullptr,
                       (float*)nullptr, 0, M, N, K, tn, ep);
    ADF_HIP_CHECK(hipGetLastError());
    return ADF_OK;
}

int32_t adf_launch_gemm16_fused(const float* A, int lda, const adf_w16* W, int M, int H, int K, int epi,
                                const adf_epi* ep_in, hipStream_t s, const adf_lift* lf) {
    adf_epi epv = *ep_in;
    const adf_epi* ep = &epv;
    if (M <= 0) return ADF_OK;
    if (K % HK != 0 || (lda & 3) || H % 64 != 0 || (epi != 3 && !W->bias_perm)) {
        adf_set_error("gemm16_fused: bad shape");
        return ADF_EINVAL;
    }
    ADF_TRY(check_a_span(epi == 3 ? 3ll * M : (long long)M, lda));
    ADF_TRY(lift_mags(A, lda, K, nullptr, 0, epi == 3 ? 3ll * M : (long long)M, lf, ep_in->rmag, &epv.rmag, s, ep_in->m_dev,
                      epi == 3 ? 3 : 1));
    const int N = 3 * H, TM = 128, TN = 192;
    const int tiles_n = N / TN;
    const int tiles_m = (M + TM - 1) / TM;
    const int tiles_m8 = (tiles_m + 7) / 8 * 8;
    dim3 grid((unsigned)(tiles_m8 * tiles_n));
    if (epi == 3) {
        const int tn = 2 * H / 128, tm8 = ((M + 63) / 64 + 7) / 8 * 8;
        static int wreg = -1;
        if (wreg < 0) { const char* e = getenv("ADF_GEMM_WREG"); wreg = (e && atoi(e) == 0) ? 0 : 1; }
        static int w8 = -1;
        if (w8 < 0) { const char* e = getenv("ADF_GEMM_W8"); w8 = (e && atoi(e) == 0) ? 0 : 1; }
        if (wreg && W->frag && w8 == 1 && (2 * H) % 256 == 0 && (K / HK) % 2 == 0)
            hipLaunchKernelGGL((adf_gemm_f16x3_kernel<0, 3, 2, 3, true, 4>), dim3((unsigned)(tm8 * (2 * H / 256))), dim3(512), 0, s,
                               A, lda, (const _Float16*)W->frag, (const _Float16*)nullptr, W->inv_scale, (const float*)nullptr,
                               (float*)nullptr, 0, M, 2 * H, K, 2 * H / 256, *ep);
        else
        hipLaunchKernelGGL((adf_gemm_f16x3_kernel<0, 3, 2, 3>), dim3((unsigned)(tm8 * tn)), dim3(256), 0, s, A, lda,
                           (const _Float16*)W->hi, (const _Float16*)W->lo, W->inv_scale, (const float*)nullptr,
                           (float*)nullptr, 0, M, 2 * H, K, tn, *ep);
        ADF_HIP_CHECK(hipGetLastError());
        return ADF_OK;
    }
    static int wf = -1;
    if (wf < 0) { const char* e = getenv("ADF_GEMM_WR_FUSED"); wf = e ? atoi(e) : 2; }
    if (wf && W->frag && (K / HK) % 2 == 0 && (wf == 2 || N % 384 == 0)) {
        const int tnw = wf == 4 ? N / 384 : tiles_n;
        dim3 gw((unsigned)(tiles_m8 * tnw));
#define LAUNCHWF(EPI_, NWN_)                                                                                                  \
        hipLaunchKernelGGL((adf_gemm_f16x3_kernel<0, 2, 3, EPI_, true, NWN_>), gw, dim3(128 * NWN_), 0, s, A, lda,            \
                           (const _Float16*)W->frag, (const _Float16*)nullptr, W->inv_scale, W->bias_perm, (float*)nullptr, 0, \
                           M, N, K, tnw, *ep)
        if (epi == 1) { if (wf == 4) LAUNCHWF(1, 4); else LAUNCHWF(1, 2); }
        else { if (wf == 4) LAUNCHWF(2, 4); else LAUNCHWF(2, 2); }
#undef LAUNCHWF
        ADF_HIP_CHECK(hipGetLastError());
        return ADF_OK;
    }
    if (epi == 1)
        hipLaunchKernelGGL((adf_gemm_f16x3_kernel<0, 2, 3, 1>), grid, dim3(256), 0, s, A, lda, (const _Float16*)W->hi,
                           (const _Float16*)W->lo, W->inv_scale, W->bias_perm, (float*)nullptr, 0, M, N, K, tiles_n, *ep);
    else
        hipLaunchKernelGGL((adf_gemm_f16x3_kernel<0, 2, 3, 2>), grid, dim3(256), 0, s, A, lda, (const _Float16*)W->hi,
                           (const _Float16*)W->lo, W->inv_scale, W->bias_perm, (float*)nullptr, 0, M, N, K, tiles_n, *ep);
    ADF_HIP_CHECK(hipGetLastError());
    return ADF_OK;
}
```

adsorbdiff_amd/csrc/message.h:

```cpp
#pragma once
#include "common.h"

typedef float f32x16 __attribute__((ext_vector_type(16)));
typedef _Float16 half8 __attribute__((ext_vector_type(8)));

#define MSG_THREADS 512
#define MSG_WAVES 8
#define MSG_COLS 192
#define MSG_LDK 136

struct MsgParams {
    const float* rec;
    const float* vec;
    const float* x;
    float* x_out;
    float* vec_out;
    const int32_t* tlist;
    int items;
    const int32_t* items_dev;
    const int32_t* nptr;
    const int32_t* e_src;
    const float4* e_geom;
    const float* wpack;
    const _Float16* wpack16;
    const float* bpack;
    const float* inv_scale;
    const float* mu;
    int N, H, R, G, nslices;
    float inv_cutoff, coeff, sarg, env_a, env_b, env_c;
    float dmu2, dmusq, cstep;
    int env_pi;
    unsigned long long* kcount;
};
```

adsorbdiff_amd/csrc/message.hip:

```cpp
#include <stdlib.h>
#include <string.h>

#include "message.h"

#ifndef MSG_ABL
#define MSG_ABL 0
#endif
#ifndef MSG_SKIP
#define MSG_SKIP 1
#endif
#ifndef MSG_EXP_NOXC
#define MSG_EXP_NOXC 0
#endif

__device__ __forceinline__ float wave_min(float v) {
#pragma unroll
    for (int o = 32; o > 0; o >>= 1) v = fminf(v, __shfl_xor(v, o));
    return v;
}
__device__ __forceinline__ float wave_max(float v) {
#pragma unroll
    for (int o = 32; o > 0; o >>= 1) v = fmaxf(v, __shfl_xor(v, o));
    return v;
}

#ifndef FWD_WAVES
#define FWD_WAVES 8
#endif
#ifndef FWD_AHEAD
#define FWD_AHEAD 4
#endif
#define FWD_THREADS (64 * FWD_WAVES)
#define MSG_WAVES_PER_SIMD (FWD_WAVES / 4)
template <bool F16, bool VZ, bool UNI>
__global__ __launch_bounds__(FWD_THREADS, MSG_WAVES_PER_SIMD) void adf_message_kernel(MsgParams p) {
    extern __shared__ __attribute__((aligned(16))) float lds[];
    const int wfloats = F16 ? (2 * MSG_COLS * MSG_LDK) / 2 : p.R * MSG_COLS;
    float* Wl = lds;
    _Float16* Wh = reinterpret_cast<_Float16*>(lds);
    _Float16* Wlo = Wh + MSG_COLS * MSG_LDK;
    float* Bl = lds + wfloats;
    float* Mu = Bl + MSG_COLS;
    float* Meta = Mu + 144;
    int* Ctr = reinterpret_cast<int*>(Meta + FWD_WAVES * 32 * 8);

    const int tid = threadIdx.x;
    const int lane = tid & 63;
    const int wave = tid >> 6;
    const int q = lane & 31;
    const int hi = lane >> 5;
    const int slice = blockIdx.x % p.nslices;
    const int worker = blockIdx.x / p.nslices;
    const int nworkers = gridDim.x / p.nslices;
    const int items = p.items_dev ? min(p.items, (int)*p.items_dev) : p.items;
    const int ngroups = (items + ADF_GROUP_NODES - 1) / ADF_GROUP_NODES;
    if (worker >= ngroups) return;
    const int H = p.H;
    const int c0 = slice * ADF_SLICE_CH;

    {
        if (F16) {
            const int R8 = p.R / 8;
            const half8* src = reinterpret_cast<const half8*>(p.wpack16 + (size_t)slice * 2 * MSG_COLS * p.R);
            const half8 zero8 = {0, 0, 0, 0, 0, 0, 0, 0};
            const _Float16* b16 = reinterpret_cast<const _Float16*>(p.bpack) + (size_t)slice * MSG_COLS * 2;
            for (int i = tid; i < 2 * MSG_COLS * 17; i += FWD_THREADS) {
                const int row = i / 17, piece = i - row * 17;
                half8 v = piece < R8 ? src[row * R8 + piece] : zero8;
                if (piece == 16 && row < MSG_COLS) { v[0] = b16[2 * row]; v[1] = b16[2 * row + 1]; }
                *reinterpret_cast<half8*>(Wh + (size_t)row * MSG_LDK + piece * 8) = v;
            }
        } else {
            const float4* src = reinterpret_cast<const float4*>(p.wpack + (size_t)slice * p.R * MSG_COLS);
            float4* dst = reinterpret_cast<float4*>(Wl);
            const int n4 = p.R * MSG_COLS / 4;
            for (int i = tid; i < n4; i += FWD_THREADS) dst[i] = src[i];
        }
        if (!F16 && tid < MSG_COLS) Bl[tid] = p.bpack[slice * MSG_COLS + tid];
        if (tid < 144) Mu[tid] = (tid < p.R ? p.mu[tid] : 2.0f) * (F16 ? p.sarg : 1.0f);
        if (tid == 0) *Ctr = 0;
    }
    __syncthreads();
    float* meta_w = Meta + wave * 32 * 8;
    const float inv_sqrt3 = 0.57735026918962576f;
    const float inv_sqrt2 = 0.70710678118654752f;
    const float out_scale = F16 ? *p.inv_scale * (1.0f / 256.0f) : 1.0f;
    const float inv_sqrt_h = out_scale / sqrtf((float)H);
    const float umax_scale = (float)(p.R - 1);
    const float coeff2 = p.coeff * 1.44269504088896341f;
    const unsigned int row_bytes = (unsigned int)p.nslices * 1280u;
    const char* recS = reinterpret_cast<const char*>(p.rec) + (size_t)slice * 1280;
    const unsigned int qA = (unsigned int)q * 16u;
    const unsigned int qP = 512u + (unsigned int)q * 4u;

    unsigned int ksteps = 0;

    typedef const __attribute__((address_space(4))) int32_t* cint_ptr;
    const cint_ptr nptr_c = (cint_ptr)p.nptr;
    const cint_ptr tlist_c = (cint_ptr)p.tlist;
    auto fetch_target = [&](int& n_out, int& o_out) -> bool {
        while (true) {
            int t = 0;
            if (lane == 0) t = atomicAdd(Ctr, 1);
            t = __builtin_amdgcn_readfirstlane(t);
            const int g = worker + (t >> 5) * nworkers;
            if (g >= ngroups) return false;
            const int e = g * ADF_GROUP_NODES + (t & 31);
            if (e < items) { o_out = e; n_out = p.tlist ? tlist_c[e] : e; return true; }
        }
    };
    auto load_block = [&](int eb, int e1, float4& geo, int& src, bool& valid) {
        const int e = eb + q;
        valid = e < e1;
        geo = make_float4(0.f, 0.f, 0.f, 0.f);
        src = 0;
        if (valid) { geo = p.e_geom[e]; src = p.e_src[e]; }
    };

    int n = 0, orow = 0, eb = 0, e1 = 0;
    bool have = fetch_target(n, orow);
    if (have) { eb = nptr_c[n]; e1 = nptr_c[n + 1]; }
    int nN = 0, oN = 0, e0N = 0, e1N = 0;
    bool haveN = have && fetch_target(nN, oN);
    if (haveN) { e0N = nptr_c[nN]; e1N = nptr_c[nN + 1]; }
    float4 geo = make_float4(0.f, 0.f, 0.f, 0.f); int src = 0; bool valid = false;
    if (have) load_block(eb, e1, geo, src, valid);
    asm volatile("" : "+v"(geo.x), "+v"(geo.y), "+v"(geo.z), "+v"(geo.w), "+v"(src));
    bool first = true;
    float sx0 = 0.f, sx1 = 0.f, sa0 = 0.f, sa1 = 0.f, sb0 = 0.f, sb1 = 0.f, sc0 = 0.f, sc1 = 0.f;
    float ra0 = 0.f, ra1 = 0.f, rb0 = 0.f, rb1 = 0.f, rc0 = 0.f, rc1 = 0.f;
    float res0 = 0.f, res1 = 0.f, res2 = 0.f, res3 = 0.f;

    while (have) {
        {
            const bool last = eb + 32 >= e1;
            float4 geoN = make_float4(0.f, 0.f, 0.f, 0.f); int srcN = 0; bool validN = false;
            if (!last) load_block(eb + 32, e1, geoN, srcN, validN);
            else if (haveN) load_block(e0N, e1N, geoN, srcN, validN);
            if (first) {
                const size_t xo = (size_t)n * H + c0 + q;
                const size_t vo = (size_t)n * 3 * H + c0 + q;
                if (hi == 0) {
                    res0 = p.x[xo]; res1 = p.x[xo + 32];
                    if (!VZ) { res2 = p.vec[vo]; res3 = p.vec[vo + 32]; }
                } else if (!VZ) {
                    res0 = p.vec[vo + H]; res1 = p.vec[vo + H + 32];
                    res2 = p.vec[vo + 2 * H]; res3 = p.vec[vo + 2 * H + 32];
                }
            }

            const float xs = geo.w * p.inv_cutoff;
            float xp = xs;
            if (p.env_pi == 5) { const float x2 = xs * xs; xp = x2 * x2 * xs; }
            else for (int i = 1; i < p.env_pi; ++i) xp *= xs;
            float env = 1.0f + p.env_a * xp + p.env_b * (xp * xs) + p.env_c * (xp * xs * xs);
            env = (xs < 1.0f && valid) ? env : 0.0f;
            __builtin_amdgcn_wave_barrier();
            if (hi == 0) {
                float* m = meta_w + q * 8;
                m[0] = __uint_as_float((unsigned int)(valid ? src : p.N) * row_bytes);
                m[1] = geo.x; m[2] = geo.y; m[3] = geo.z;
            }
            __builtin_amdgcn_fence(__ATOMIC_RELEASE, "wavefront");
            __builtin_amdgcn_wave_barrier();
            const float u = xs * umax_scale;
            const int nvalid = __builtin_amdgcn_readfirstlane(min(32, e1 - eb));
            const float umin = __int_as_float(__builtin_amdgcn_readlane(__float_as_int(u), 0));
            const float umax = __int_as_float(__builtin_amdgcn_readlane(__float_as_int(u), max(nvalid, 1) - 1));
            int klo, khi;
            if (nvalid <= 0) {
                klo = 0; khi = 16;
            } else if (F16) {
                klo = max(0, (int)floorf(umin) - 5) & ~7;
                khi = min(p.R, (int)ceilf(umax) + 6);
                khi = klo + ((khi - klo + 15) & ~15);
                if (khi > 128) { klo -= khi - 128; khi = 128; }
            } else {
                klo = max(0, (int)floorf(umin) - 7) & ~1;
                khi = min(p.R, ((int)ceilf(umax) + 8 + 1) & ~1);
            }
            klo = __builtin_amdgcn_readfirstlane(klo);
            khi = __builtin_amdgcn_readfirstlane(khi);
            ksteps += (khi - klo) * (VZ && F16 ? 4 : 6);

#define ROW_OF(r) ((r & 3) + 8 * (r >> 2) + 4 * hi)
#define DECL(r)                                                                                 \
    const float* m##r = meta_w + ROW_OF(r) * 8;                                                 \
    float4 ga0##r, ga1##r;                                      \
    float gz0##r, gz1##r;
#define GATHER(r)                                                                               \
    {                                                                                           \
    const unsigned int o##r = __float_as_uint(m##r[0]);                                         \
    if (MSG_EXP_NOXC) { gz0##r = 1.0f; gz1##r = 2.0f; } else {                                 \
    gz0##r = *reinterpret_cast<const float*>(recS + (size_t)(o##r + qP));                       \
    gz1##r = *reinterpret_cast<const float*>(recS + (size_t)(o##r + qP) + 640); }               \
    if (MSG_EXP_NOXC == 2) { ga0##r = make_float4(1.f, 2.f, 3.f, 4.f); ga1##r = ga0##r; }      \
    else if (!VZ) {                                                                             \
        ga0##r = *reinterpret_cast<const float4*>(recS + (size_t)(o##r + qA));                  \
        ga1##r = *reinterpret_cast<const float4*>(recS + (size_t)(o##r + qA) + 640);            \
    } else {                                                                                    \
        ga0##r = make_float4(0.f, 0.f, 0.f, *reinterpret_cast<const float*>(recS + (size_t)(o##r + qA) + 12)); \
        ga1##r = make_float4(0.f, 0.f, 0.f, *reinterpret_cast<const float*>(recS + (size_t)(o##r + qA) + 652)); \
    }                                                                                           \
    }
#define CONSUME(r)                                                                              \
    {                                                                                           \
        const float ux = m##r[1], uy = m##r[2], uz = m##r[3];                                   \
        const float t3 = gz0##r * acc[4][r];                                                    \
        sx0 += ga0##r.w * acc[0][r];                                                            \
        if (!VZ) { sa0 += ga0##r.x * acc[2][r]; sb0 += ga0##r.y * acc[2][r]; sc0 += ga0##r.z * acc[2][r]; } \
        ra0 += t3 * ux; rb0 += t3 * uy; rc0 += t3 * uz;                                         \
        const float u3 = gz1##r * acc[5][r];                                                    \
        sx1 += ga1##r.w * acc[1][r];                                                            \
        if (!VZ) { sa1 += ga1##r.x * acc[3][r]; sb1 += ga1##r.y * acc[3][r]; sc1 += ga1##r.z * acc[3][r]; } \
        ra1 += u3 * ux; rb1 += u3 * uy; rc1 += u3 * uz;                                         \
    }
            DECL(0) DECL(1) DECL(2) DECL(3) DECL(4) DECL(5) DECL(6) DECL(7)
            DECL(8) DECL(9) DECL(10) DECL(11) DECL(12) DECL(13) DECL(14) DECL(15)
            GATHER(0) GATHER(1)
#if FWD_AHEAD == 4
            GATHER(2) GATHER(3)
#endif

            const float env256 = env * 256.0f;
            f32x16 acc[6];
            if (F16) {
                half8 aone = {0, 0, 0, 0, 0, 0, 0, 0};
                if (hi == 0) { aone[0] = (_Float16)256.0f; aone[1] = (_Float16)256.0f; }
                const f32x16 zero16 = {0.f, 0.f, 0.f, 0.f, 0.f, 0.f, 0.f, 0.f, 0.f, 0.f, 0.f, 0.f, 0.f, 0.f, 0.f, 0.f};
#pragma unroll
                for (int b = 0; b < 6; ++b) {
                    if (VZ && (b == 2 || b == 3)) continue;
                    const half8 bb = *reinterpret_cast<const half8*>(Wh + (size_t)(b * 32 + q) * MSG_LDK + 128);
                    acc[b] = __builtin_amdgcn_mfma_f32_32x32x16_f16(aone, bb, zero16, 0, 0, 0);
                }
            } else {
#pragma unroll
                for (int b = 0; b < 6; ++b) {
                    const float bv = Bl[b * 32 + q];
#pragma unroll
                    for (int r = 0; r < 16; ++r) acc[b][r] = bv;
                }
            }
            if (F16) {
                const float xsq = xs * p.sarg;
                auto gen_a = [&](int k0, half8& ah, half8& al) {
                    if constexpr (UNI) {
                        const float t0 = xsq - Mu[k0 + 8 * hi];
                        float a = env256 * __builtin_amdgcn_exp2f(-(t0 * t0));
                        float r = __builtin_amdgcn_exp2f(fminf(p.dmu2 * t0 - p.dmusq, 64.0f));
                        float av[8];
#pragma unroll
                        for (int j = 0; j < 8; ++j) {
                            av[j] = a;
                            a *= r;
                            r *= p.cstep;
                        }
#pragma unroll
                        for (int j = 0; j < 8; j += 2) {
                            typedef __fp16 h2_t __attribute__((ext_vector_type(2)));
                            const h2_t hh = __builtin_amdgcn_cvt_pkrtz(av[j], av[j + 1]);
                            const h2_t ll = __builtin_amdgcn_cvt_pkrtz(av[j] - (float)hh[0], av[j + 1] - (float)hh[1]);
                            ah[j] = (_Float16)hh[0]; ah[j + 1] = (_Float16)hh[1];
                            al[j] = (_Float16)ll[0]; al[j + 1] = (_Float16)ll[1];
                        }
                    } else {
                        const float4 mu0 = *reinterpret_cast<const float4*>(Mu + k0 + 8 * hi);
                        const float4 mu1 = *reinterpret_cast<const float4*>(Mu + k0 + 8 * hi + 4);
                        const float mus[8] = {mu0.x, mu0.y, mu0.z, mu0.w, mu1.x, mu1.y, mu1.z, mu1.w};
#pragma unroll
                        for (int j = 0; j < 8; ++j) {
                            const float dm = xsq - mus[j];
                            const float a = env256 * __builtin_amdgcn_exp2f(-(dm * dm));
                            const _Float16 h = (_Float16)a;
                            ah[j] = h;
                            al[j] = (_Float16)(a - (float)h);
                        }
                    }
                };
                int k0 = klo;
                if (MSG_ABL != 1)
                do {
                    half8 ah, al;
                    gen_a(k0, ah, al);
                    const _Float16* wh = Wh + (size_t)q * MSG_LDK + k0 + 8 * hi;
                    const _Float16* wl = Wlo + (size_t)q * MSG_LDK + k0 + 8 * hi;
#pragma unroll
                    for (int b = 0; b < 6; ++b) {
                        if (VZ && (b == 2 || b == 3)) continue;
                        const half8 bh = *reinterpret_cast<const half8*>(wh + b * 32 * MSG_LDK);
                        const half8 bl = *reinterpret_cast<const half8*>(wl + b * 32 * MSG_LDK);
                        acc[b] = __builtin_amdgcn_mfma_f32_32x32x16_f16(al, bh, acc[b], 0, 0, 0);
                        acc[b] = __builtin_amdgcn_mfma_f32_32x32x16_f16(ah, bl, acc[b], 0, 0, 0);
                        acc[b] = __builtin_amdgcn_mfma_f32_32x32x16_f16(ah, bh, acc[b], 0, 0, 0);
                    }
                    k0 += 16;
                } while (k0 < khi);
            } else {
                int k2 = klo;
                do {
                    const int k = k2 + hi;
                    const float dm = xs - Mu[k];
                    const float a = env * __builtin_amdgcn_exp2f(coeff2 * (dm * dm));
                    const float* wrow = Wl + k * MSG_COLS + q;
#pragma unroll
                    for (int b = 0; b < 6; ++b)
                        acc[b] = __builtin_amdgcn_mfma_f32_32x32x2f32(a, wrow[b * 32], acc[b], 0, 0, 0);
                    k2 += 2;
                } while (k2 < khi);
            }
#if MSG_ABL == 2
#pragma unroll
            for (int b = 0; b < 6; ++b) asm volatile("" :: "v"(acc[b]));
            sx0 += m0[1];
#elif FWD_AHEAD == 2
            GATHER(2) GATHER(3)
            CONSUME(0) CONSUME(1)
            GATHER(4) GATHER(5)
            CONSUME(2) CONSUME(3)
            GATHER(6) GATHER(7)
            CONSUME(4) CONSUME(5)
            if (nvalid <= 16) {
                CONSUME(6) CONSUME(7)
            } else {
                GATHER(8) GATHER(9)
                CONSUME(6) CONSUME(7)
                GATHER(10) GATHER(11)
                CONSUME(8) CONSUME(9)
                GATHER(12) GATHER(13)
                CONSUME(10) CONSUME(11)
                GATHER(14) GATHER(15)
                CONSUME(12) CONSUME(13)
                CONSUME(14) CONSUME(15)
            }
#elif MSG_SKIP
            GATHER(4) GATHER(5) GATHER(6) GATHER(7)
            CONSUME(0) CONSUME(1) CONSUME(2) CONSUME(3)
            if (nvalid <= 16) {
                CONSUME(4) CONSUME(5) CONSUME(6) CONSUME(7)
            } else {
                GATHER(8) GATHER(9) GATHER(10) GATHER(11)
                CONSUME(4) CONSUME(5) CONSUME(6) CONSUME(7)
#if MSG_SKIP >= 2
                if (nvalid <= 24) {
                    CONSUME(8) CONSUME(9) CONSUME(10) CONSUME(11)
                } else
#endif
                {
                    GATHER(12) GATHER(13) GATHER(14) GATHER(15)
                    CONSUME(8) CONSUME(9) CONSUME(10) CONSUME(11)
                    CONSUME(12) CONSUME(13) CONSUME(14) CONSUME(15)
                }
            }
#else
            GATHER(4) GATHER(5) GATHER(6) GATHER(7)
            CONSUME(0) CONSUME(1) CONSUME(2) CONSUME(3)
            GATHER(8) GATHER(9) GATHER(10) GATHER(11)
            CONSUME(4) CONSUME(5) CONSUME(6) CONSUME(7)
            GATHER(12) GATHER(13) GATHER(14) GATHER(15)
            CONSUME(8) CONSUME(9) CONSUME(10) CONSUME(11)
            CONSUME(12) CONSUME(13) CONSUME(14) CONSUME(15)
#endif
#undef GATHER
#undef DECL
#undef CONSUME
#undef ROW_OF
            if (last) {
                sx0 *= out_scale; sx1 *= out_scale;
                sa0 = (sa0 * inv_sqrt3 + ra0) * inv_sqrt_h; sa1 = (sa1 * inv_sqrt3 + ra1) * inv_sqrt_h;
                sb0 = (sb0 * inv_sqrt3 + rb0) * inv_sqrt_h; sb1 = (sb1 * inv_sqrt3 + rb1) * inv_sqrt_h;
                sc0 = (sc0 * inv_sqrt3 + rc0) * inv_sqrt_h; sc1 = (sc1 * inv_sqrt3 + rc1) * inv_sqrt_h;
                sx0 += __shfl_xor(sx0, 32); sx1 += __shfl_xor(sx1, 32);
                sa0 += __shfl_xor(sa0, 32); sa1 += __shfl_xor(sa1, 32);
                sb0 += __shfl_xor(sb0, 32); sb1 += __shfl_xor(sb1, 32);
                sc0 += __shfl_xor(sc0, 32); sc1 += __shfl_xor(sc1, 32);
                const size_t xo = (size_t)orow * H + c0 + q;
                const size_t vo = (size_t)orow * 3 * H + c0 + q;
                if (hi == 0) {
                    p.x_out[xo] = (res0 + sx0) * inv_sqrt2;
                    p.x_out[xo + 32] = (res1 + sx1) * inv_sqrt2;
                    p.vec_out[vo] = res2 + sa0;
                    p.vec_out[vo + 32] = res3 + sa1;
                } else {
                    p.vec_out[vo + H] = res0 + sb0;
                    p.vec_out[vo + H + 32] = res1 + sb1;
                    p.vec_out[vo + 2 * H] = res2 + sc0;
                    p.vec_out[vo + 2 * H + 32] = res3 + sc1;
                }
                sx0 = sx1 = sa0 = sa1 = sb0 = sb1 = sc0 = sc1 = 0.f;
                ra0 = ra1 = rb0 = rb1 = rc0 = rc1 = 0.f;
                res0 = res1 = res2 = res3 = 0.f;
                have = haveN;
                n = nN; orow = oN; eb = e0N; e1 = e1N;
                first = true;
                if (have) {
                    haveN = fetch_target(nN, oN);
                    if (haveN) { e0N = nptr_c[nN]; e1N = nptr_c[nN + 1]; }
                }
            } else {
                eb += 32;
                first = false;
            }
            geo = geoN; src = srcN; valid = validN;
        }
    }
    if (p.kcount && lane == 0) atomicAdd(p.kcount, (unsigned long long)ksteps);
}

__global__ void adf_pack_rbf_kernel(const float* __restrict__ w, const float* __restrict__ b, float* wpack,
                                    float* bpack, int H, int R) {
    const int nslices = H / ADF_SLICE_CH;
    const int total = nslices * R * MSG_COLS;
    for (int i = blockIdx.x * blockDim.x + threadIdx.x; i < total; i += gridDim.x * blockDim.x) {
        const int col = i % MSG_COLS;
        const int k = (i / MSG_COLS) % R;
        const int slice = i / (MSG_COLS * R);
        const int part = col / 64, j = (col >> 5) & 1, qq = col & 31;
        const int ch = slice * ADF_SLICE_CH + 32 * j + qq;
        wpack[i] = w[(size_t)(part * H + ch) * R + k];
        if (k == 0) bpack[slice * MSG_COLS + col] = b[part * H + ch];
    }
}

__global__ void adf_pack_rbf16_kernel(const float* __restrict__ w, const float* __restrict__ b,
                                      const unsigned int* absmax_bits, _Float16* wpack16, float* bpack16,
                                      float* inv_scale, int H, int R) {
    const float amax = __uint_as_float(*absmax_bits);
    int e = 0;
    if (amax > 0.f) (void)frexpf(amax, &e);
    const float scale = ldexpf(1.0f, 10 - e);
    if (blockIdx.x == 0 && threadIdx.x == 0) *inv_scale = 1.0f / scale;
    const int nslices = H / ADF_SLICE_CH;
    const int total = nslices * MSG_COLS * R;
    for (int i = blockIdx.x * blockDim.x + threadIdx.x; i < total; i += gridDim.x * blockDim.x) {
        const int k = i % R;
        const int col = (i / R) % MSG_COLS;
        const int slice = i / (R * MSG_COLS);
        const int part = col / 64, j = (col >> 5) & 1, qq = col & 31;
        const int ch = slice * ADF_SLICE_CH + 32 * j + qq;
        const float v = w[(size_t)(part * H + ch) * R + k] * scale;
        const _Float16 h = (_Float16)v;
        const size_t base = (size_t)slice * 2 * MSG_COLS * R;
        wpack16[base + (size_t)col * R + k] = h;
        wpack16[base + (size_t)(MSG_COLS + col) * R + k] = (_Float16)(v - (float)h);
        if (k == 0) {
            const float bv = b[part * H + ch] * scale;
            const _Float16 bh = (_Float16)bv;
            _Float16* o = reinterpret_cast<_Float16*>(bpack16 + slice * MSG_COLS + col);
            o[0] = bh; o[1] = (_Float16)(bv - (float)bh);
        }
    }
}

__global__ void adf_absmax_kernel(const float* __restrict__ w, long long n, unsigned int* out_bits);

__global__ void adf_pack_records_kernel(const float* __restrict__ xh, const float* __restrict__ vec,
                                        float* __restrict__ rec, int N, int H, int vec_is_zero) {
    const int ng = H / 32;
    const long long total = (long long)N * ng * 32;
    for (long long t = (long long)blockIdx.x * blockDim.x + threadIdx.x; t < total;
         t += (long long)gridDim.x * blockDim.x) {
        const int qq = (int)(t & 31);
        const int g = (int)((t >> 5) % ng);
        const long long n = t / (32LL * ng);
        const int c = 32 * g + qq;
        const float* xr = xh + (size_t)n * 3 * H;
        const float xa = xr[c], xb = xr[H + c], xc = xr[2 * H + c];
        float* out = rec + ((size_t)n * ng + g) * 160;
        if (!vec_is_zero) {
            const float* vr = vec + (size_t)n * 3 * H;
            reinterpret_cast<float4*>(out)[qq] = make_float4(vr[c] * xb, vr[H + c] * xb, vr[2 * H + c] * xb, xa);
        } else {
            reinterpret_cast<float4*>(out)[qq] = make_float4(0.f, 0.f, 0.f, xa);
        }
        out[128 + qq] = xc;
    }
}

int32_t adf_pack_records(adf_painn* h, int N, const float* xh, const float* vec, bool vec_is_zero, hipStream_t s,
                         float* rec) {
    const int H = h->hp.hidden_channels;
    long long blocks = ((long long)N * H + 255) / 256;
    if (blocks > 256 * 16) blocks = 256 * 16;
    hipLaunchKernelGGL(adf_pack_records_kernel, dim3((unsigned)blocks), dim3(256), 0, s, xh, vec, rec ? rec : h->rec, N, H,
                       vec_is_zero ? 1 : 0);
    ADF_HIP_CHECK(hipGetLastError());
    return ADF_OK;
}

static size_t msg_lds_bytes(int R, bool f16) {
    const size_t w = f16 ? (size_t)2 * MSG_COLS * MSG_LDK * 2 : sizeof(float) * (size_t)R * MSG_COLS;
    return w + sizeof(float) * (MSG_COLS + 144 + FWD_WAVES * 32 * 8) + 16;
}

int32_t adf_pack_rbf_layer(adf_painn* h, int l, hipStream_t s) {
    const int H = h->hp.hidden_channels, R = h->hp.num_rbf;
    const size_t per_layer = (size_t)(H / ADF_SLICE_CH) * R * MSG_COLS;
    const size_t per_layer_b = (size_t)(H / ADF_SLICE_CH) * MSG_COLS;
    hipLaunchKernelGGL(adf_pack_rbf_kernel, dim3(256), dim3(256), 0, s, h->layer[l].rbf_w, h->layer[l].rbf_b,
                       h->rbf_pack + l * per_layer, h->rbf_bias_pack + l * per_layer_b, H, R);
    ADF_HIP_CHECK(hipMemsetAsync(h->w16_scratch, 0, sizeof(unsigned int), s));
    hipLaunchKernelGGL(adf_absmax_kernel, dim3(64), dim3(256), 0, s, h->layer[l].rbf_w, (long long)3 * H * R,
                       h->w16_scratch);
    hipLaunchKernelGGL(adf_absmax_kernel, dim3(8), dim3(256), 0, s, h->layer[l].rbf_b, (long long)3 * H,
                       h->w16_scratch);
    hipLaunchKernelGGL(adf_pack_rbf16_kernel, dim3(256), dim3(256), 0, s, h->layer[l].rbf_w, h->layer[l].rbf_b,
                       h->w16_scratch, reinterpret_cast<_Float16*>(h->rbf_pack16) + l * 2 * per_layer,
                       h->rbf_bias_pack16 + l * per_layer_b, h->rbf_scales + l, H, R);
    ADF_HIP_CHECK(hipGetLastError());
    return ADF_OK;
}

int32_t adf_pack_rbf(adf_painn* h, hipStream_t s) {
    const int H = h->hp.hidden_channels, R = h->hp.num_rbf;
    {
        float mu[128];
        ADF_HIP_CHECK(hipMemcpyAsync(mu, h->rbf_offset, sizeof(float) * R, hipMemcpyDeviceToHost, s));
        ADF_HIP_CHECK(hipStreamSynchronize(s));
        bool uni = true;
        for (int k = 0; k < R; ++k) uni = uni && fabsf(mu[k] - (float)k / (float)(R - 1)) <= 2e-7f;
        const char* e = getenv("ADF_MSG_RBF");
        h->rbf_uniform = uni && !(e && strcmp(e, "direct") == 0);
    }
    for (int l = 0; l < h->hp.num_layers; ++l) ADF_TRY(adf_pack_rbf_layer(h, l, s));
    ADF_HIP_CHECK(hipGetLastError());
    {
#define SET_LDS(F16_, VZ_, UNI_)                                                                              \
    ADF_HIP_CHECK(hipFuncSetAttribute(reinterpret_cast<const void*>(adf_message_kernel<F16_, VZ_, UNI_>),     \
                                      hipFuncAttributeMaxDynamicSharedMemorySize, (int)msg_lds_bytes(128, F16_)))
        SET_LDS(false, false, false); SET_LDS(false, true, false); SET_LDS(true, false, false); SET_LDS(true, true, false);
        SET_LDS(true, false, true); SET_LDS(true, true, true);
#undef SET_LDS
    }
    return ADF_OK;
}

int32_t adf_message_impl(adf_painn* h, int layer, int N, const float* x, const float* xh, const float* vec,
                         float* x_out, float* vec_out, bool vec_is_zero, hipStream_t s, const int32_t* tlist,
                         int n_targets, const float* rec, const int32_t* n_targets_dev) {
    const int H = h->hp.hidden_channels, R = h->hp.num_rbf;
    if ((unsigned long long)(N + 1) * 5ull * H * sizeof(float) >= (1ull << 32)) {
        adf_set_error("message kernel uses 32-bit byte offsets into the node tables: N=%d is too large, split the batch", N);
        return ADF_EOOM;
    }
    MsgParams p;
    p.rec = rec ? rec : h->rec; p.vec = vec; p.x = x; p.x_out = x_out; p.vec_out = vec_out;
    p.nptr = h->nptr; p.e_src = h->e_src; p.e_geom = h->e_geom;
    p.nslices = H / ADF_SLICE_CH;
    const bool f16 = !h->msg_f32;
    p.wpack = h->rbf_pack + (size_t)layer * p.nslices * R * MSG_COLS;
    p.wpack16 = reinterpret_cast<const _Float16*>(h->rbf_pack16) + (size_t)layer * 2 * p.nslices * R * MSG_COLS;
    p.bpack = (f16 ? h->rbf_bias_pack16 : h->rbf_bias_pack) + (size_t)layer * p.nslices * MSG_COLS;
    p.inv_scale = h->rbf_scales + layer;
    p.mu = h->rbf_offset;
    p.N = N; p.H = H; p.R = R;
    p.tlist = tlist; p.items = tlist ? n_targets : N; p.items_dev = tlist ? n_targets_dev : nullptr;
    if (p.items <= 0) return ADF_OK;
    p.G = (p.items + ADF_GROUP_NODES - 1) / ADF_GROUP_NODES;
    p.inv_cutoff = 1.0f / h->hp.cutoff;
    const double step = 1.0 / (R - 1);
    p.coeff = (float)(-0.5 / (step * step));
    p.sarg = (float)sqrt(0.5 / (step * step) * 1.4426950408889634);
    const double pe = (double)h->hp.envelope_exponent;
    p.env_pi = h->hp.envelope_exponent;
    p.env_a = (float)(-(pe + 1) * (pe + 2) / 2);
    p.env_b = (float)(pe * (pe + 2));
    p.env_c = (float)(-pe * (pe + 1) / 2);
    p.kcount = h->prof_on ? h->kcount : nullptr;
    int workers = h->num_cus / p.nslices;
    if (workers < 1) workers = 1;
    if (workers > p.G) workers = p.G;
    dim3 grid((unsigned)(workers * p.nslices));
#define LAUNCH_MSG(F16_, VZ_, UNI_)                                                                        \
    hipLaunchKernelGGL((adf_message_kernel<F16_, VZ_, UNI_>), grid, dim3(FWD_THREADS), msg_lds_bytes(R, F16_), s, p)
    {
        const double d = sqrt(0.5 / (step * step) * 1.4426950408889634) * step;
        p.dmu2 = (float)(2.0 * d); p.dmusq = (float)(d * d); p.cstep = (float)exp2(-2.0 * d * d);
    }
    if (f16 && h->rbf_uniform) { if (vec_is_zero) LAUNCH_MSG(true, true, true); else LAUNCH_MSG(true, false, true); }
    else if (f16) { if (vec_is_zero) LAUNCH_MSG(true, true, false); else LAUNCH_MSG(true, false, false); }
    else { if (vec_is_zero) LAUNCH_MSG(false, true, false); else LAUNCH_MSG(false, false, false); }
#undef LAUNCH_MSG
    ADF_HIP_CHECK(hipGetLastError());
    return ADF_OK;
}
```

Measured before the change: 241.0.

## Emit per-slice row magnitude partials from message and vp epilogues to skip rowmag passes

The message kernel and the vp GEMM epilogue now also write per-row partial absolute maxima for each channel slice. The following f16x3 GEMMs reduce these partials when computing their per-row lift scales, so they no longer need separate rowmag kernel launches that re-read the activations. The cost is small extra reductions and stores in the producer epilogues, three new scratch buffers, and plumbing across several kernels.

```diff
diff --git a/adsorbdiff_amd/csrc/api.hip b/adsorbdiff_amd/csrc/api.hip
--- a/adsorbdiff_amd/csrc/api.hip
+++ b/adsorbdiff_amd/csrc/api.hip
@@ -155,6 +155,8 @@
         h->lift_on = !(el && strcmp(el, "0") == 0);
         const char* e2 = getenv("ADF_MSG");
         h->msg_f32 = e2 ? strcmp(e2, "f32") == 0 : h->gemm_f32;
+        const char* ep = getenv("ADF_MAG_PARTS");
+        h->mag_parts = !(ep && strcmp(ep, "0") == 0);
     }
     if (st == ADF_OK) st = dev_alloc(&h->kcount, 8);
     if (st == ADF_OK && hipMemset(h->kcount, 0, 8 * sizeof(unsigned long long)) != hipSuccess) st = ADF_EHIP;
@@ -182,6 +184,7 @@
 static void free_workspaces(adf_painn* h) {
     void* ptrs[] = {h->nbr_cnt, h->nbr_src, h->nbr_shift, h->deg, h->nptr, h->cursor, h->img_cnt, h->sys_slow, h->scan_tmp,
                     h->e_src, h->e_geom, h->x, h->vecA, h->vecB, h->y, h->xh, h->vv, h->cat, h->dot, h->sys, h->rec, h->lift.buf, h->mag_a, h->mag_b, h->mag_v3,
+                    h->part_x, h->part_v, h->part_v2,
                     h->cache_d2, h->cache_cid, h->cache_cnt, h->prev_nptr, h->prev_src, h->prev_geom};
     for (void* p : ptrs)
         if (p) (void)hipFree(p);
@@ -191,6 +194,7 @@
     h->e_geom = nullptr;
     h->x = h->vecA = h->vecB = h->y = h->xh = h->vv = h->cat = h->dot = h->sys = h->rec = nullptr;
     h->lift.buf = h->mag_a = h->mag_b = h->mag_v3 = nullptr; h->lift.cap = 0; h->mag_v3_valid = false;
+    h->part_x = h->part_v = h->part_v2 = nullptr;
     h->cache_d2 = nullptr; h->cache_cid = nullptr; h->cache_cnt = nullptr; h->cache_valid = false;
     h->capN = h->capB = h->capE = 0;
 }
@@ -360,6 +364,9 @@
     ALLOC(mag_a, capN);
     ALLOC(mag_b, capN);
     ALLOC(mag_v3, capN * 3);
+    ALLOC(part_x, capN * (H / ADF_SLICE_CH));
+    ALLOC(part_v, capN * 3 * (H / ADF_SLICE_CH));
+    ALLOC(part_v2, capN * (H / 32));
 #undef ALLOC
     h->lift.cap = st == ADF_OK ? capN * 3 : 0;
     if (st != ADF_OK) { free_workspaces(h); return st; }
@@ -519,19 +526,27 @@
     return ADF_OK;
 }
 
+static bool use_mag_parts(const adf_painn* h) {
+    const int H = h->hp.hidden_channels;
+    return h->mag_parts && h->lift_on && !h->gemm_f32 && H % 256 == 0;
+}
+
 static int32_t message_layer(adf_painn* h, int l, int N, const float* x, const float* vec, float* x_out,
                              float* vec_out, bool vec_is_zero, hipStream_t s, const int32_t* tlist = nullptr,
                              int n_targets = 0, float* rec = nullptr, bool records_ready = false) {
     if (!records_ready) ADF_TRY(make_records(h, l, N, x, vec, vec_is_zero, rec, nullptr, s));
     adf_prof_begin(h, ADF_PROF_MESSAGE, s);
+    const bool parts = use_mag_parts(h) && (tlist ? n_targets : N) <= h->capN;
     const int32_t st = adf_message_impl(h, l, N, x, h->xh, vec, x_out, vec_out, vec_is_zero, s, tlist, n_targets, rec,
-                                        tlist ? h->rows_dev : nullptr);
+                                        tlist ? h->rows_dev : nullptr, parts ? h->part_x : nullptr,
+                                        parts ? h->part_v : nullptr);
     adf_prof_end(h, s);
     return st;
 }
 
-static int32_t update_layer(adf_painn* h, int l, int N, float* x, float* vec, hipStream_t s) {
+static int32_t update_layer(adf_painn* h, int l, int N, float* x, float* vec, hipStream_t s, bool parts_ready = false) {
     const int H = h->hp.hidden_channels;
+    const bool parts = parts_ready && use_mag_parts(h) && N <= h->capN;
     const adf_layer_weights& w = h->layer[l];
     adf_prof_begin(h, ADF_PROF_NODE, s);
     if (h->gemm_f32) {
@@ -542,6 +557,7 @@
         adf_epi ep = {};
         ep.v1 = h->vv; ep.dotw = h->dot; ep.cat = h->cat; ep.H = H; ep.m_dev = h->rows_dev;
         const adf_lift* lf = h->lift_on ? &h->lift : nullptr;
+        if (parts) { ep.rpart = h->part_v; ep.rpart_n = H / ADF_SLICE_CH; ep.part_out = h->part_v2; }
         ADF_TRY(adf_launch_gemm16_fused(vec, H, &w.vp_16, N, H, H, 3, &ep, s, lf));
         if (use_fused_mlp(h, N)) {
             const float* rm = nullptr;
@@ -557,8 +573,9 @@
             adf_prof_end(h, s);
             return stf;
         }
+        const adf_mag_parts xp = {h->part_x, H / ADF_SLICE_CH, h->part_v2, H / 32};
         ADF_TRY(adf_launch_gemm16(x, H, &w.xv0_16, w.xv0_b, h->y, H, N, H, 2 * H, 1, s, h->cat, H, lf, nullptr,
-                                  h->lift_on ? h->mag_b : nullptr, h->rows_dev));
+                                  h->lift_on ? h->mag_b : nullptr, h->rows_dev, 0, nullptr, 0, parts ? &xp : nullptr));
     }
     int32_t st;
     if (h->gemm_f32) {
@@ -735,7 +752,7 @@
         if (whole) {
             ADF_TRY(message_layer(h, l, N, h->incX[l], vin, h->incX[l + 1], h->incV[l + 1], l == 0, s, nullptr, 0,
                                   h->incR[l], true));
-            ADF_TRY(update_layer(h, l, N, h->incX[l + 1], h->incV[l + 1], s));
+            ADF_TRY(update_layer(h, l, N, h->incX[l + 1], h->incV[l + 1], s, true));
             if (l + 1 < L)
                 ADF_TRY(make_records(h, l + 1, N, h->incX[l + 1], h->incV[l + 1], false, h->incR[l + 1], nullptr, s));
             continue;
@@ -744,7 +761,7 @@
         const int ncap = h->inc_sync ? n_seen : N;
         h->rows_dev = h->inc_cnt + l;
         int32_t st = message_layer(h, l, N, h->incX[l], vin, h->x, h->vecB, l == 0, s, list, ncap, h->incR[l], true);
-        if (st == ADF_OK) st = update_layer(h, l, ncap, h->x, h->vecB, s);
+        if (st == ADF_OK) st = update_layer(h, l, ncap, h->x, h->vecB, s, true);
         if (st == ADF_OK) {
             adf_prof_begin(h, ADF_PROF_NODE, s);
             st = adf_inc_scatter_rows(h->x, list, ncap, H, h->incX[l + 1], s, h->rows_dev);
@@ -830,7 +847,7 @@
             if (l == 0) ADF_TRY(message_layer(h, 0, N, h->x, vin, h->x, vout, true, s, nullptr, 0, rec0, rec0_ready));
             else
             ADF_TRY(message_layer(h, l, N, h->x, vin, h->x, vout, l == 0, s));
-            ADF_TRY(update_layer(h, l, N, h->x, vout, s));
+            ADF_TRY(update_layer(h, l, N, h->x, vout, s, true));
             float* t = vin; vin = vout; vout = t;
         }
         adf_prof_begin(h, ADF_PROF_HEADS, s);
@@ -856,12 +873,12 @@
         if (l == 0) ADF_TRY(message_layer(h, 0, N, h->x, vin, h->x, vout, true, s, nullptr, 0, rec0, rec0_ready));
         else
         ADF_TRY(message_layer(h, l, N, h->x, vin, h->x, vout, l == 0, s));
-        ADF_TRY(update_layer(h, l, N, h->x, vout, s));
+        ADF_TRY(update_layer(h, l, N, h->x, vout, s, true));
         float* t = vin; vin = vout; vout = t;
     }
     ADF_TRY(message_layer(h, L - 1, N, h->x, vin, h->sub_x, h->sub_vec, L == 1, s, out_idx, n_out,
                           L == 1 ? rec0 : nullptr, L == 1 && rec0_ready));
-    ADF_TRY(update_layer(h, L - 1, n_out, h->sub_x, h->sub_vec, s));
+    ADF_TRY(update_layer(h, L - 1, n_out, h->sub_x, h->sub_vec, s, true));
     adf_prof_begin(h, ADF_PROF_HEADS, s);
     for (int hd = 0; hd < heads; ++hd) {
         ADF_TRY(adf_head_forward(h, hd, n_out, h->sub_x, h->sub_vec, h->sub_f, s));
diff --git a/adsorbdiff_amd/csrc/common.h b/adsorbdiff_amd/csrc/common.h
--- a/adsorbdiff_amd/csrc/common.h
+++ b/adsorbdiff_amd/csrc/common.h
@@ -57,6 +57,10 @@
     int K1;
     const int32_t* row_map;
     const float* rmag;
+    const float* rpart;
+    const float* rpart2;
+    int rpart_n, rpart2_n;
+    float* part_out;
     unsigned int* out_mag;
     const int32_t* m_dev;
     int accumulate;
@@ -68,6 +72,12 @@
 struct adf_lift {
     float* buf;
     long long cap;
+};
+struct adf_mag_parts {
+    const float* p1;
+    int n1;
+    const float* p2;
+    int n2;
 };
 struct adf_layer_weights {
     const float *ln_w, *ln_b, *xp0_w, *xp0_b, *xp2_w, *xp2_b, *rbf_w, *rbf_b;
@@ -107,6 +117,10 @@
     float *mag_a, *mag_b;
     float* mag_v3;
     bool mag_v3_valid;
+    bool mag_parts;
+    float* part_x;
+    float* part_v;
+    float* part_v2;
 
     int64_t capN, capB, capE;
     int32_t* nbr_cnt;
@@ -191,7 +205,8 @@
                           int N, int K, int act_ssilu, hipStream_t s, const float* A2 = nullptr, int K1 = 0,
                           const adf_lift* lf = nullptr, const float* premag = nullptr, float* out_mag = nullptr,
                           const int32_t* m_dev = nullptr, int accumulate = 0,
-                          const float* gate = nullptr, int gate_ld = 0);
+                          const float* gate = nullptr, int gate_ld = 0,
+                          const adf_mag_parts* parts = nullptr);
 int32_t adf_launch_rowmag(const float* A, int lda, int K1, const float* A2, int K2, long long M, float* mag, hipStream_t s,
                           const int32_t* m_dev = nullptr, int m_mul = 1);
 int32_t adf_split_weight(const float* w, long long n, adf_w16* out, unsigned int* scratch_bits, hipStream_t s,
@@ -223,7 +238,8 @@
 int32_t adf_message_impl(adf_painn* h, int layer, int N, const float* x, const float* xh, const float* vec,
                          float* x_out, float* vec_out, bool vec_is_zero, hipStream_t s,
                          const int32_t* tlist = nullptr, int n_targets = 0, const float* rec = nullptr,
-                         const int32_t* n_targets_dev = nullptr);
+                         const int32_t* n_targets_dev = nullptr,
+                         float* xpart = nullptr, float* vpart = nullptr);
 int32_t adf_pack_rbf(adf_painn* h, hipStream_t s);
 int32_t adf_pack_rbf_layer(adf_painn* h, int l, hipStream_t s);
 int32_t adf_pack_records(adf_painn* h, int N, const float* xh, const float* vec, bool vec_is_zero, hipStream_t s,
diff --git a/adsorbdiff_amd/csrc/gemm16.hip b/adsorbdiff_amd/csrc/gemm16.hip
--- a/adsorbdiff_amd/csrc/gemm16.hip
+++ b/adsorbdiff_amd/csrc/gemm16.hip
@@ -42,6 +42,24 @@
     v = fmaxf(v, ADF_ROR(1));
 #undef ADF_ROR
     return v;
+}
+
+__device__ __forceinline__ float adf_epi_rowmag(const adf_epi& ep, unsigned int r) {
+    if (ep.rmag) return ep.rmag[r];
+    float m = 0.f;
+    const float4* p = reinterpret_cast<const float4*>(ep.rpart + (size_t)r * ep.rpart_n);
+    for (int k = 0; k < ep.rpart_n / 4; ++k) {
+        const float4 v = p[k];
+        m = fmaxf(m, fmaxf(fmaxf(v.x, v.y), fmaxf(v.z, v.w)));
+    }
+    if (ep.rpart2) {
+        const float4* p2 = reinterpret_cast<const float4*>(ep.rpart2 + (size_t)r * ep.rpart2_n);
+        for (int k = 0; k < ep.rpart2_n / 4; ++k) {
+            const float4 v = p2[k];
+            m = fmaxf(m, fmaxf(fmaxf(v.x, v.y), fmaxf(v.z, v.w)));
+        }
+    }
+    return m;
 }
 
 template <int ACT, int MI, int NJ, int EPI, bool WR = false, int NWN = 2>
@@ -96,9 +114,9 @@
         const unsigned int grow = global_row(row);
         a_goff[i] = (grow * (unsigned int)lda + kq * 4) * 4u;
         a_off[i] = row * HLD + kq * 4;
-        a_rs[i] = ep.rmag ? adf_pow2_lift(ep.rmag[grow]) : 1.0f;
-    }
-    if (tid < TM) rinv[tid] = ep.rmag ? 1.0f / adf_pow2_lift(ep.rmag[global_row(tid)]) : 1.0f;
+        a_rs[i] = (ep.rmag || ep.rpart) ? adf_pow2_lift(adf_epi_rowmag(ep, grow)) : 1.0f;
+    }
+    if (tid < TM) rinv[tid] = (ep.rmag || ep.rpart) ? 1.0f / adf_pow2_lift(adf_epi_rowmag(ep, global_row(tid))) : 1.0f;
     const char* const A1b = reinterpret_cast<const char*>(A);
     const char* const A2b = reinterpret_cast<const char*>(ep.A2) - (size_t)ep.K1 * 4;
     int w_src[NJ];
@@ -432,9 +450,16 @@
         for (int it = 0; it < 4; ++it) {
             const int lr = it * 8 + (lane >> 3), c4 = lane & 7;
             const int n = a0 + lr, c = 32 * g + 4 * c4;
+            const float4 dv_ = *reinterpret_cast<const float4*>(T + lr * TLD3 + 4 * c4);
+            const float4 nv_ = *reinterpret_cast<const float4*>(T + lr * TLD3 + 32 + 4 * c4);
+            if (ep.part_out) {
+                float mg = fmaxf(fmaxf(fabsf(nv_.x), fabsf(nv_.y)), fmaxf(fabsf(nv_.z), fabsf(nv_.w)));
+                mg = fmaxf(mg, __shfl_xor(mg, 1));
+                mg = fmaxf(mg, __shfl_xor(mg, 2));
+                mg = fmaxf(mg, __shfl_xor(mg, 4));
+                if (c4 == 0 && n < M) ep.part_out[(size_t)n * (H / 32) + g] = mg;
+            }
             if (n < M) {
-                const float4 dv_ = *reinterpret_cast<const float4*>(T + lr * TLD3 + 4 * c4);
-                const float4 nv_ = *reinterpret_cast<const float4*>(T + lr * TLD3 + 32 + 4 * c4);
                 if (G16_ABL & 1) { asm volatile("" :: "v"(dv_.x), "v"(nv_.w)); } else {
                 *reinterpret_cast<float4*>(ep.dotw + (size_t)n * H + c) = dv_;
                 *reinterpret_cast<float4*>(ep.cat + (size_t)n * H + c) = nv_;
@@ -615,8 +640,17 @@
 }
 
 static int32_t lift_mags(const float* A, int lda, int K1, const float* A2, int K2, long long rows, const adf_lift* lf,
-                         const float* premag, const float** out, hipStream_t s, const int32_t* m_dev = nullptr, int m_mul = 1) {
+                         const float* premag, const float** out, hipStream_t s, const int32_t* m_dev = nullptr, int m_mul = 1,
+                         const adf_mag_parts* parts = nullptr, adf_epi* ep = nullptr) {
     *out = premag;
+    if (!premag && lf && parts && parts->p1) {
+        if ((parts->n1 & 3) || (parts->p2 && (parts->n2 & 3)) || parts->n1 <= 0) {
+            adf_set_error("gemm16: partial maxima per row must come in multiples of 4"); return ADF_EINVAL;
+        }
+        ep->rpart = parts->p1; ep->rpart_n = parts->n1;
+        ep->rpart2 = parts->p2; ep->rpart2_n = parts->p2 ? parts->n2 : 0;
+        return ADF_OK;
+    }
     if (!premag && lf && lf->buf) {
         if (rows > lf->cap) { adf_set_error("gemm16: lift scratch holds %lld rows, need %lld", lf->cap, rows); return ADF_EINVAL; }
         ADF_TRY(adf_launch_rowmag(A, lda, K1, A2, K2, rows, lf->buf, s, m_dev, m_mul));
@@ -681,7 +715,7 @@
 int32_t adf_launch_gemm16(const float* A, int lda, const adf_w16* W, const float* bias, float* C, int ldc, int M,
                           int N, int K, int act_ssilu, hipStream_t s, const float* A2, int K1, const adf_lift* lf,
                           const float* premag, float* out_mag, const int32_t* m_dev, int accumulate, const float* gate,
-                          int gate_ld) {
+                          int gate_ld, const adf_mag_parts* parts) {
     if (M <= 0) return ADF_OK;
     if (K % HK != 0 || (lda & 3) || (A2 && (K1 <= 0 || K1 % HK != 0 || K1 >= K))) {
         adf_set_error("gemm16: K=%d (K1=%d) must be multiples of %d and lda a multiple of 4", K, K1, HK);
@@ -699,7 +733,7 @@
     ep.A2 = A2; ep.K1 = A2 ? K1 : 0; ep.m_dev = m_dev; ep.accumulate = accumulate;
     ep.gate = gate; ep.gate_ld = gate_ld;
     if (gate && ((N | ldc) & 3)) { adf_set_error("gemm16: the gate epilogue needs N and ldc multiples of 4"); return ADF_EINVAL; }
-    ADF_TRY(lift_mags(A, lda, A2 ? K1 : K, A2, A2 ? K - K1 : 0, M, lf, premag, &ep.rmag, s, m_dev, 1));
+    ADF_TRY(lift_mags(A, lda, A2 ? K1 : K, A2, A2 ? K - K1 : 0, M, lf, premag, &ep.rmag, s, m_dev, 1, parts, &ep));
     if (out_mag) {
         ADF_HIP_CHECK(hipMemsetAsync(out_mag, 0, sizeof(float) * (size_t)M, s));
         ep.out_mag = reinterpret_cast<unsigned int*>(out_mag);
@@ -768,8 +802,14 @@
         return ADF_EINVAL;
     }
     ADF_TRY(check_a_span(epi == 3 ? 3ll * M : (long long)M, lda));
+    if (ep_in->rpart) {
+        if ((ep_in->rpart_n & 3) || ep_in->rpart_n <= 0 || (ep_in->rpart2 && (ep_in->rpart2_n & 3))) {
+            adf_set_error("gemm16_fused: partial maxima per row must come in multiples of 4"); return ADF_EINVAL;
+        }
+    } else
     ADF_TRY(lift_mags(A, lda, K, nullptr, 0, epi == 3 ? 3ll * M : (long long)M, lf, ep_in->rmag, &epv.rmag, s, ep_in->m_dev,
                       epi == 3 ? 3 : 1));
+    if (epv.part_out && (epi != 3 || H % 32 != 0)) { adf_set_error("gemm16_fused: part_out is an EPI 3 output"); return ADF_EINVAL; }
     const int N = 3 * H, TM = 128, TN = 192;
     const int tiles_n = N / TN;
     const int tiles_m = (M + TM - 1) / TM;
diff --git a/adsorbdiff_amd/csrc/message.h b/adsorbdiff_amd/csrc/message.h
--- a/adsorbdiff_amd/csrc/message.h
+++ b/adsorbdiff_amd/csrc/message.h
@@ -30,5 +30,7 @@
     float inv_cutoff, coeff, sarg, env_a, env_b, env_c;
     float dmu2, dmusq, cstep;
     int env_pi;
+    float* xpart;
+    float* vpart;
     unsigned long long* kcount;
 };
diff --git a/adsorbdiff_amd/csrc/message.hip b/adsorbdiff_amd/csrc/message.hip
--- a/adsorbdiff_amd/csrc/message.hip
+++ b/adsorbdiff_amd/csrc/message.hip
@@ -32,6 +32,16 @@
 #endif
 #define FWD_THREADS (64 * FWD_WAVES)
 #define MSG_WAVES_PER_SIMD (FWD_WAVES / 4)
+__device__ __forceinline__ float adf_msg_row16_max(float v) {
+#define ADF_ROR(n_) __int_as_float(__builtin_amdgcn_update_dpp(0, __float_as_int(v), 0x120 + (n_), 0xf, 0xf, false))
+    v = fmaxf(v, ADF_ROR(8));
+    v = fmaxf(v, ADF_ROR(4));
+    v = fmaxf(v, ADF_ROR(2));
+    v = fmaxf(v, ADF_ROR(1));
+#undef ADF_ROR
+    return v;
+}
+
 template <bool F16, bool VZ, bool UNI>
 __global__ __launch_bounds__(FWD_THREADS, MSG_WAVES_PER_SIMD) void adf_message_kernel(MsgParams p) {
     extern __shared__ __attribute__((aligned(16))) float lds[];
@@ -376,16 +386,37 @@
                 sc0 += __shfl_xor(sc0, 32); sc1 += __shfl_xor(sc1, 32);
                 const size_t xo = (size_t)orow * H + c0 + q;
                 const size_t vo = (size_t)orow * 3 * H + c0 + q;
+                float u0, u1, w0, w1;
                 if (hi == 0) {
-                    p.x_out[xo] = (res0 + sx0) * inv_sqrt2;
-                    p.x_out[xo + 32] = (res1 + sx1) * inv_sqrt2;
-                    p.vec_out[vo] = res2 + sa0;
-                    p.vec_out[vo + 32] = res3 + sa1;
+                    u0 = (res0 + sx0) * inv_sqrt2; u1 = (res1 + sx1) * inv_sqrt2;
+                    w0 = res2 + sa0; w1 = res3 + sa1;
+                    p.x_out[xo] = u0;
+                    p.x_out[xo + 32] = u1;
+                    p.vec_out[vo] = w0;
+                    p.vec_out[vo + 32] = w1;
                 } else {
-                    p.vec_out[vo + H] = res0 + sb0;
-                    p.vec_out[vo + H + 32] = res1 + sb1;
-                    p.vec_out[vo + 2 * H] = res2 + sc0;
-                    p.vec_out[vo + 2 * H + 32] = res3 + sc1;
+                    u0 = res0 + sb0; u1 = res1 + sb1;
+                    w0 = res2 + sc0; w1 = res3 + sc1;
+                    p.vec_out[vo + H] = u0;
+                    p.vec_out[vo + H + 32] = u1;
+                    p.vec_out[vo + 2 * H] = w0;
+                    p.vec_out[vo + 2 * H + 32] = w1;
+                }
+                if (p.xpart) {
+                    float mu = adf_msg_row16_max(fmaxf(fabsf(u0), fabsf(u1)));
+                    float mw = adf_msg_row16_max(fmaxf(fabsf(w0), fabsf(w1)));
+                    mu = fmaxf(mu, __int_as_float(__builtin_amdgcn_update_dpp(__float_as_int(mu), __float_as_int(mu), 0x142, 0xa, 0xf, false)));
+                    mw = fmaxf(mw, __int_as_float(__builtin_amdgcn_update_dpp(__float_as_int(mw), __float_as_int(mw), 0x142, 0xa, 0xf, false)));
+                    if (q == 31) {
+                        const size_t r3 = (size_t)orow * 3 * p.nslices + slice;
+                        if (hi == 0) {
+                            p.xpart[(size_t)orow * p.nslices + slice] = mu;
+                            p.vpart[r3] = mw;
+                        } else {
+                            p.vpart[r3 + p.nslices] = mu;
+                            p.vpart[r3 + 2 * p.nslices] = mw;
+                        }
+                    }
                 }
                 sx0 = sx1 = sa0 = sa1 = sb0 = sb1 = sc0 = sc1 = 0.f;
                 ra0 = ra1 = rb0 = rb1 = rc0 = rc1 = 0.f;
@@ -537,7 +568,7 @@
 
 int32_t adf_message_impl(adf_painn* h, int layer, int N, const float* x, const float* xh, const float* vec,
                          float* x_out, float* vec_out, bool vec_is_zero, hipStream_t s, const int32_t* tlist,
-                         int n_targets, const float* rec, const int32_t* n_targets_dev) {
+                         int n_targets, const float* rec, const int32_t* n_targets_dev, float* xpart, float* vpart) {
     const int H = h->hp.hidden_channels, R = h->hp.num_rbf;
     if ((unsigned long long)(N + 1) * 5ull * H * sizeof(float) >= (1ull << 32)) {
         adf_set_error("message kernel uses 32-bit byte offsets into the node tables: N=%d is too large, split the batch", N);
@@ -567,6 +598,8 @@
     p.env_b = (float)(pe * (pe + 2));
     p.env_c = (float)(-pe * (pe + 1) / 2);
     p.kcount = h->prof_on ? h->kcount : nullptr;
+    p.xpart = xpart; p.vpart = vpart;
+    if ((xpart == nullptr) != (vpart == nullptr)) { adf_set_error("message: partial maxima need both buffers"); return ADF_EINVAL; }
     int workers = h->num_cus / p.nslices;
     if (workers < 1) workers = 1;
     if (workers > p.G) workers = p.G;
```

After: 242.0, median of 6. No clear change (+0.4%).
